# linto-ai/ssak

Hardware: AMD Instinct MI355X
Metric: utterances/sec (16 kHz, 10 s) Wav2Vec2-base CTC train step (higher is better)
Workload: dtype bf16; 1 GPU; Wav2Vec2-base CTC fine-tune step, bf16, synthetic 10 s @16 kHz utterances (BASELINE.json configs[1]; DP over xGMI for n_gpus>1 = configs[2]); per_gpu_batch=32, global_batch=32, samples_per_utt=160000, frames=499, frozen_feature_encoder=True, regularisers=script defaults (dropout/layerdrop/specaugment on), parallelism=dp1

## Files before the change

include/ssak_hip.h:

```cpp
#ifndef SSAK_HIP_H
#define SSAK_HIP_H
#include <stddef.h>
#include <stdint.h>

#ifdef __cplusplus
extern "C" {
#endif

#define SSAK_OK 0
#define SSAK_ERR_INVALID (-1)
#define SSAK_ERR_LAUNCH (-2)
#define SSAK_ERR_STATE (-3)

#define SSAK_REDUCTION_SUM 0
#define SSAK_REDUCTION_MEAN 1

int ssak_version(void);
const char* ssak_last_error(void);

size_t ssak_wave_normalize_workspace_bytes(int B, int T);
int ssak_wave_normalize(const float* in, const int32_t* lens, int B, int T, float* out, int32_t* mask,
                        void* workspace, size_t workspace_bytes, void* stream);

size_t ssak_logmel_table_floats(void);
// ... 277 lines not shown
#define SSAK_CLS_SITE_INPUT 4
#define SSAK_CLS_SITE_HIDDEN 5
int ssak_cls_head_fwd(const float* pooled, const float* W1, const float* b1, const float* W2, const float* b2, int B, int H, int C,
                      float drop_p, uint64_t seed, int training, float* act, float* logits, void* stream);
size_t ssak_cls_head_bwd_workspace_bytes(int B, int H, int C);
int ssak_cls_head_bwd(const float* dlogits, const float* pooled, const float* act, const float* W1, const float* W2, int B, int H, int C,
                      float drop_p, uint64_t seed, int training, float* dW1, float* db1, float* dW2, float* db2, float* dpooled,
                      void* workspace, size_t workspace_bytes, void* stream);
int ssak_cls_softmax_ce(const float* logits, const int32_t* labels, const int32_t* labels_host , int B, int C, float grad_scale,
                        float* probs, float* loss, float* dlogits, void* stream);

int ssak_dec_embed(const void* embed_tokens, const void* embed_positions, const int32_t* ids, const int32_t* ids_host , int B, int L,
                   int D, int V, int max_positions, int pos_offset, void* out, void* stream);
int ssak_dec_attention_fwd(const void* q, long ldq, const void* k, long ldk, const void* v, long ldv, int Lk, const int32_t* klens,
                           const int32_t* klens_host , int B, int Lq, int nh, int head_dim, int causal, int q_offset, void* ctx,
                           void* stream);
int ssak_token_logprobs(const void* logits, int dtype, int R, int V, long ldv, const int32_t* targets, const int32_t* targets_host ,
                        const int32_t* allowed, const int32_t* allowed_host , int n_allowed, float* lse, float* logprob,
                        int32_t* argmax, float* probs, void* stream);

size_t ssak_dec_attention_step_workspace_bytes(int B, int nh, int n_split);
int ssak_dec_attention_step(const void* q, long ldq, const void* k, long ldk, long k_batch_stride, const void* v, long ldv,
                            long v_batch_stride, int n_keys, const int32_t* klens, int B, int nh, int head_dim, int n_split, void* workspace,
                            size_t workspace_bytes, void* ctx, void* stream);
int ssak_dec_greedy_step(const float* logits, long ldv, int B, int V, const uint8_t* suppress, const uint8_t* begin_suppress, int first,
                         const void* embed_tokens, const void* embed_positions, int D, int max_positions, int next_pos, int eos_id, int pad_id,
                         uint8_t* finished, int32_t* n_unfinished, int32_t* tokens, float* logprobs, long ldt, int t, void* h_next,
                         void* stream);
int ssak_dec_timestamp_step(const float* logits, long ldv, int B, int V, const uint8_t* suppress, const uint8_t* begin_suppress, int first,
                            int ts_begin, int no_timestamps_id, int max_initial, const void* embed_tokens, const void* embed_positions, int D,
                            int max_positions, int next_pos, int eos_id, int pad_id, uint8_t* finished, int32_t* n_unfinished,
                            int32_t* tokens, float* logprobs, long ldt, int t, int32_t* ts_last, void* h_next, void* stream);
int ssak_dec_beam_topk(const float* logits, long ldv, int B, int nb, int V, const uint8_t* suppress, const uint8_t* begin_suppress, int first,
                       int timestamps, int ts_begin, int no_timestamps_id, int max_initial, int eos_id, const int32_t* tokens, long ldt, int t,
                       const int32_t* ts_last, const uint8_t* done, int K, int32_t* cand_token, float* cand_logprob, void* stream);
int ssak_dec_beam_select(const int32_t* cand_token, const float* cand_logprob, int B, int nb, int K, int V, float* sum_logprob, int32_t* src,
                         int32_t* tokens, float* logprobs, long ldt, int t, int32_t* ts_last, int ts_begin, int32_t* fin_tokens,
                         float* fin_logprobs, int32_t* fin_len, float* fin_sum, int32_t* n_fin, uint8_t* done, int32_t* n_unfinished,
                         const void* embed_tokens, const void* embed_positions, int D, int max_positions, int next_pos, int eos_id, int pad_id,
                         void* h_next, void* stream);
int ssak_dec_kv_reorder(void* cache, const int32_t* src, int layers, int B, int nb, int cap, int width, long layer_stride, long row_stride,
                        long key_stride, int row_lo, int row_hi, void* stream);
int ssak_dec_attention_step_grouped(const void* q, long ldq, const void* k, long ldk, long k_batch_stride, const void* v, long ldv,
                                    long v_batch_stride, int n_keys, const int32_t* klens, int B, int nh, int head_dim, int n_split, int group,
                                    void* workspace, size_t workspace_bytes, void* ctx, void* stream);
int ssak_layernorm_fwd(const void* y, const void* res, const float* gamma, const float* beta, void* r_out, void* out, int M, int C,
                       float eps, int dtype, void* stream);

int ssak_debug_dropout_mask(uint64_t seed, uint32_t site, float p, long rows, int cols, uint8_t* keep, float* scale_out ,
                            void* stream);
int ssak_debug_attention_dropout_mask(uint64_t seed, uint32_t site, float p, int B, int nh, int F, uint8_t* keep, void* stream);

int ssak_debug_layernorm_fwd(const void* y, const void* res, const float* gamma, const float* beta, void* r_out, void* out, float* mean,
                             float* rstd, int M, int C, float eps, uint64_t seed, uint32_t pre_site, float pre_p, uint32_t mid_site,
                             float mid_p, uint32_t post_site, float post_p, int post_gelu, int dtype, void* stream);
size_t ssak_debug_layernorm_bwd_workspace_bytes(int C);
int ssak_debug_layernorm_bwd(const void* g1, const void* g2, const void* r, const float* mean, const float* rstd, const float* gamma,
                             const void* g_res, void* dr, void* dy, float* dgamma, float* dbeta, float* dy_colsum,
                             const float* post_gelu_beta, int M, int C, uint64_t seed, uint32_t pre_site, float pre_p, uint32_t mid_site,
                             float mid_p, uint32_t post_site, float post_p, int queued, int dtype, void* workspace,
                             size_t workspace_bytes, void* stream);
int ssak_debug_softmax_fwd(const void* S, void* P, void* Pd, const int32_t* klens, int rows, int cols, int ld, int rows_per_batch,
                           uint64_t seed, uint32_t site, float p, int dtype, void* stream);
int ssak_debug_softmax_bwd(const void* dPd, const void* P, void* dS, int rows, int cols, int ld, uint64_t seed, uint32_t site, float p,
                           int dtype, void* stream);
int ssak_debug_gelu(const float* x, long n, float* y, float* dydx, int dtype, void* stream);

int ssak_test_attn_adapter_fwd(const void* y, const void* res, const float* ln_g, const float* ln_b, const void* w1, const float* b1,
                               const void* w2, const float* b2, const float* next_g, const float* next_b, void* r_out, void* out,
                               float* mean, float* rstd, int M, int H, int A, float eps_adapter, float eps_next, int dtype,
                               void* stream);

int ssak_debug_posconv_prepare(const float* g, const float* v, void* wf, void* wb, float* norms, int H, int G, int K, int dtype,
                               void* stream);
int ssak_debug_posconv_pack(const void* h, void* pg, int B, int F, int H, int G, int K, int dtype, void* stream);
size_t ssak_debug_posconv_workspace_bytes(int B, int F, int H, int G, int K);
int ssak_debug_posconv_direct(const void* h, const void* w, const float* bias, void* out, void* pre, int B, int F, int H, int G, int K,
                              int row0, int gelu, void* workspace, size_t workspace_bytes, void* stream);
int ssak_debug_posconv_wgrad(const void* h, const void* dpre, float* dwf, int B, int F, int H, int G, int K, void* workspace,
                             size_t workspace_bytes, void* stream);
int ssak_debug_posconv_weight_bwd(const float* dwf, const float* g, const float* v, float* norms, float* dg, float* dv, int H, int G,
                                  int K, void* stream);

size_t ssak_debug_conv0_bwd_workspace_bytes(int B, int T, int C);
int ssak_debug_conv0_bwd(const float* x, const float* w, const float* gamma, const float* beta, const void* dy, const double* sums,
                         float* dw, float* dgamma, float* dbeta, int B, int T, int C, int dtype, void* workspace, size_t workspace_bytes,
                         void* stream);
size_t ssak_debug_conv0_wgrad_workspace_bytes(int B, int C, int ksize);
int ssak_debug_conv0_wgrad(const void* d, const float* x, float* dw, int B, int T, int C, int ksize, int stride, int dtype, void* workspace,
                           size_t workspace_bytes, void* stream);
int ssak_debug_conv0_bias(const float* x, const float* w, const float* bias, void* out, int B, int T, int C, int dtype, void* stream);
int ssak_debug_col2im(const void* dxcol, void* dx, int B, int Tin, int Tout, int C, int k, int s, int dtype, void* stream);
int ssak_debug_sum_slabs(const float* slabs, int nb, long n, float* out, void* stream);
int ssak_debug_conv_weight_rearrange(const float* w, void* out, int Co, int Ci, int k, int dtype, void* stream);
int ssak_debug_conv_wgrad_unrearrange(const float* dwr, float* g, int Co, int Ci, int k, void* stream);
int ssak_debug_col2im_k3s2(const void* dxcol, const void* pre, void* out, int B, int F, int Tin, int RS1, int H, int dtype, void* stream);
int ssak_debug_mel_to_cl(const float* mel, void* cl, int B, int C, int T, int RS, int lead, int dtype, void* stream);
int ssak_debug_add_rowvec(const void* x, const void* pos, void* out, int B, int F, int H, int dtype, void* stream);
int ssak_debug_copy_rows_padded(const void* src, void* dst, int B, int F, int RS, int H, int dtype, void* stream);

#ifdef __cplusplus
}
#endif
#endif
```

ssak_amd/csrc/api.cpp:

```cpp
#include <stdarg.h>
#include <stdio.h>

#include <string.h>

#include <mutex>
#include <vector>

#include "kernels.h"

static thread_local char g_err[512] = "";

void ssak_set_error(const char* fmt, ...) {
  va_list ap;
  va_start(ap, fmt);
  vsnprintf(g_err, sizeof(g_err), fmt, ap);
  va_end(ap);
}

extern "C" int ssak_version(void) { return 630; }
extern "C" const char* ssak_last_error(void) { return g_err; }

#include <atomic>
#include <map>
namespace {
struct ProfRec {
  hipEvent_t e0, e1;
  int slot;
  double work;
};
struct ProfStream {
  int mode = 0;
  std::vector<char> want;
  std::vector<ProfRec> recs;
};
struct ProfKey {
  int dev;
  hipStream_t st;
  bool operator<(const ProfKey& o) const { return dev != o.dev ? dev < o.dev : st < o.st; }
};
std::mutex g_prof_mu;
std::map<ProfKey, ProfStream> g_prof_streams;
std::atomic<int> g_prof_active{0};
std::vector<hipEvent_t> g_event_pool;
ProfKey prof_key(hipStream_t st) {
  int dev = 0;
  (void)hipGetDevice(&dev);
  return ProfKey{dev, st};
}
hipEvent_t prof_event() {
  if (!g_event_pool.empty()) {
    hipEvent_t e = g_event_pool.back();
    g_event_pool.pop_back();
    return e;
  }
  hipEvent_t e;
  (void)hipEventCreate(&e);
  return e;
}
struct SlotInfo {
  char name[112];
  int bound;
};
SlotInfo g_slots[PROF_MAX_SLOTS];
int g_nslots = 0;
std::mutex g_slot_mu;
int register_locked(const char* name, int bound) {
  for (int i = 0; i < g_nslots; ++i)
    if (!strcmp(g_slots[i].name, name)) return i;
  if (g_nslots >= PROF_MAX_SLOTS) return PROF_MAX_SLOTS - 1;
  snprintf(g_slots[g_nslots].name, sizeof(g_slots[g_nslots].name), "%s", name);
  g_slots[g_nslots].bound = bound;
  return g_nslots++;
}
void register_classes() {
  static const struct {
    const char* name;
    int bound;
  } kClasses[PROF_CLASS_SLOTS] = {
      {"attn_fwd_kernel (fused attention forward)", SSAK_BOUND_MFMA},
      {"attn_bwd_dq_kernel + attn_bwd_dkv_kernel (fused attention backward)", SSAK_BOUND_MFMA},
      {"ln_fwd_kernel (residual + dropout + LayerNorm)", SSAK_BOUND_HBM},
      {"ln_bwd_kernel (LayerNorm backward + column partials)", SSAK_BOUND_HBM},
      {"conv0_moments_kernel + conv0_channel_stats_kernel + conv0_mfma_kernel (conv0 + GroupNorm + GELU)", SSAK_BOUND_HBM},
      {"adamw_kernel (clip + AdamW + bf16 shadow)", SSAK_BOUND_HBM},
      {"sumsq_kernel (gradient norm)", SSAK_BOUND_HBM},
      {"ctc_lsm + ctc_lat + ctc_grad (CTC loss + gradient)", SSAK_BOUND_LATENCY},
      {"norm_stats + norm_apply (waveform normalise)", SSAK_BOUND_HBM},
      {"row / element-wise helpers (pack, SpecAugment, casts, column sums, GELU', adds, reductions)", SSAK_BOUND_HBM},
      {"positional-conv weight-norm prepare / backward", SSAK_BOUND_HBM},
      {"softmax fwd / bwd (unfused attention fallback)", SSAK_BOUND_HBM},
      {"posconv_direct_kernel (grouped positional convolution forward / input gradient)", SSAK_BOUND_MFMA},
      {"posconv_wgrad_kernel + posconv_wgrad_sum_kernel (grouped positional convolution weight gradient)", SSAK_BOUND_MFMA},
      {"stft_fft_mel_kernel + logmel_finalize_kernel (Whisper log-mel features)", SSAK_BOUND_HBM},
  };
  if (g_nslots == 0)
    for (int i = 0; i < PROF_CLASS_SLOTS; ++i) register_locked(kClasses[i].name, kClasses[i].bound);
}
}

int ssak_prof_register(const char* name, int bound) {
  std::lock_guard<std::mutex> lock(g_slot_mu);
  register_classes();
// ... 87 lines not shown
```

ssak_amd/csrc/conv_frontend.hip:

```cpp
#include <cstdlib>

#include "kernels.h"

namespace {

constexpr int KS0 = 10, ST0 = 5;
constexpr int FR_STATS = 1024, FR_APPLY = 128;

template <typename OT, bool APPLY, int FR0>
__global__ __launch_bounds__(256) void conv0_kernel(const float* __restrict__ x, const float* __restrict__ w,
                                                    const float* __restrict__ gamma, const float* __restrict__ beta,
                                                    OT* __restrict__ out, double* __restrict__ stats,
                                                    const double* __restrict__ sums, int T, int T0, int C) {
  constexpr int NS0 = (FR0 - 1) * ST0 + KS0;
  __shared__ float xs[NS0];
  __shared__ float red[256][9];
  const int b = blockIdx.y;
  const int f0 = blockIdx.x * FR0;
  const int nq = C >> 2;
  const int fl = 256 / nq;
  const int q = threadIdx.x % nq, fli = threadIdx.x / nq;
  const int nfr = min(FR0, T0 - f0);
  const float* xb = x + (size_t)b * T;
  for (int i = threadIdx.x; i < NS0; i += 256) {
// ... 648 lines not shown
  }
  float* out = partial + ((size_t)b * gridDim.x + blk) * C * ksize;
  const int c2 = threadIdx.x;
  if (c2 < C / 2)
#pragma unroll
    for (int k = 0; k < 10; ++k)
      if (k < ksize) {
        out[(2 * c2) * ksize + k] = acc[0][k];
        out[(2 * c2 + 1) * ksize + k] = acc[1][k];
      }
}
__global__ void conv0_wgrad_sum_kernel(const float* __restrict__ partial, int nslab, int n, float* __restrict__ dw) {
  const int e = blockIdx.x * blockDim.x + threadIdx.x;
  if (e >= n) return;
  float s = 0.f;
  for (int k = 0; k < nslab; ++k) s += partial[(size_t)k * n + e];
  dw[e] += s;
}

}

size_t k_conv0_wgrad_scratch_floats(int B, int C, int ksize) { return (size_t)B * C0W_BLOCKS_PER_UTT * C * ksize; }

template <typename DT>
int k_conv0_wgrad_t(const DT* d, const float* x, float* dw, float* scratch, int B, int T, int T0, int C, int ksize, int stride,
                    hipStream_t st) {
  SSAK_REQUIRE(ksize <= 10 && stride * 64 + ksize <= 64 * 5 + 16 && C <= 512 && (C & 1) == 0,
               "conv0_wgrad: kernel %d / stride %d / C %d outside what is built (k <= 10, stride <= 5, C <= 512)", ksize, stride, C);
  conv0_wgrad_kernel<DT><<<dim3(C0W_BLOCKS_PER_UTT, B), 256, 0, st>>>(d, x, scratch, T, T0, C, ksize, stride);
  SSAK_LAUNCH_CHECK();
  conv0_wgrad_sum_kernel<<<ssak_cdiv(C * ksize, 256), 256, 0, st>>>(scratch, B * C0W_BLOCKS_PER_UTT, C * ksize, dw);
  SSAK_LAUNCH_CHECK();
  return SSAK_OK;
}

size_t k_conv0_stats_doubles(int B, int T0, int C) {
  return (size_t)B * 2 * C + (size_t)B * ssak_cdiv(T0, FR_STATS) * std::max(2 * C, NMOM);
}

template <typename OT>
int k_conv0_gn_gelu_t(const float* x, const float* w, const float* gamma, const float* beta, OT* out, double* stats,
                      int B, int T, int T0, int C, int ksize, int stride, hipStream_t st, bool raw_input) {
  SSAK_REQUIRE(ksize == KS0 && stride == ST0, "conv0: only kernel 10 / stride 5 is built (got %d/%d)", ksize, stride);
  SSAK_REQUIRE((C & 3) == 0 && C <= 1024 && 256 % (C / 4) == 0, "conv0: C=%d must divide into 256 threads as quads", C);
  SSAK_REQUIRE(T0 == (T - KS0) / ST0 + 1 && T0 > 0, "conv0: T0 mismatch");
  const int nblk = ssak_cdiv(T0, FR_STATS);
  ProfScope prof_scope(PROF_CONV0, (double)B * ((double)T * 4.0 + (double)T0 * C * sizeof(OT)), st);
  double* sums = stats;
  double* partial = stats + (size_t)B * 2 * C;
  conv0_moments_kernel<<<dim3(nblk, B), 256, 0, st>>>(x, T, T0, partial);
  SSAK_LAUNCH_CHECK();
  conv0_channel_stats_kernel<<<dim3(ssak_cdiv(C, 256), B), 256, 0, st>>>(partial, nblk, w, C, sums, T, T0, raw_input ? 1 : 0);
  SSAK_LAUNCH_CHECK();
  if constexpr (sizeof(OT) == 2) {
    if (C == 512) {
      conv0_mfma_kernel<<<dim3(ssak_cdiv(T0, C0M_FR * C0M_SUB), B), 256, 0, st>>>(x, w, gamma, beta, (bf16*)out, sums, T, T0);
      SSAK_LAUNCH_CHECK();
      return SSAK_OK;
    }
  }
  conv0_kernel<OT, true, FR_APPLY><<<dim3(ssak_cdiv(T0, FR_APPLY), B), 256, 0, st>>>(x, w, gamma, beta, out, nullptr, sums, T, T0, C);
  SSAK_LAUNCH_CHECK();
  return SSAK_OK;
}

template <typename OT>
int k_conv0_bias_t(const float* x, const float* w, const float* bias, OT* out, int B, int T, int T0, int C, int ksize,
                   int stride, hipStream_t st) {
  SSAK_REQUIRE(ksize == KS0 && stride == ST0, "conv0: only kernel 10 / stride 5 is built (got %d/%d)", ksize, stride);
  SSAK_REQUIRE((C & 3) == 0 && C <= 1024 && 256 % (C / 4) == 0, "conv0: C=%d must divide into 256 threads as quads", C);
  ProfScope prof_scope(PROF_CONV0, (double)B * ((double)T * 4.0 + (double)T0 * C * sizeof(OT)), st);
  conv0_bias_kernel<OT><<<dim3(ssak_cdiv(T0, FR_APPLY), B), 256, 0, st>>>(x, w, bias, out, T, T0, C);
  SSAK_LAUNCH_CHECK();
  return SSAK_OK;
}

template <typename OT>
int k_conv_weight_rearrange_t(const float* w, OT* out, int Co, int Ci, int k, hipStream_t st) {
  conv_w_rearrange_kernel<OT><<<min(2048, ssak_cdiv((long)Co * Ci * k, 256)), 256, 0, st>>>(w, out, Co, Ci, k);
  SSAK_LAUNCH_CHECK();
  return SSAK_OK;
}

template <typename OT>
int k_posconv_prepare_t(const float* g, const float* v, OT* w_fwd, OT* w_bwd, float* norms, int H, int G, int K,
                        hipStream_t st) {
  SSAK_REQUIRE(K <= 1024 && H % G == 0 && ((H / G) & 7) == 0, "posconv: K=%d <= 1024 and (H/G)=%d %% 8 == 0 required", K, H / G);
  const int cg = H / G;
  float* partial = norms + 2 * K;
  ProfScope prof_scope(PROF_POSCONV_W, (double)H * cg * K * 8.0, st);
  posconv_colnorm_kernel<<<H, ((K + 63) / 64) * 64, 0, st>>>(v, nullptr, H / cg, K, cg, partial);
  SSAK_LAUNCH_CHECK();
  posconv_colnorm_finalize_kernel<<<ssak_cdiv(K, 64), 1024, 0, st>>>(partial, H, K, norms);
  SSAK_LAUNCH_CHECK();
  SSAK_REQUIRE((size_t)cg * (K + 1) * sizeof(float) <= 64 * 1024, "posconv: (H/G) x K slab does not fit in LDS");
  posconv_materialize_kernel<OT><<<2 * H, 256, (size_t)cg * (K + 1) * sizeof(float), st>>>(g, v, norms, w_fwd, w_bwd, H, cg, K);
  SSAK_LAUNCH_CHECK();
  return SSAK_OK;
}

int k_posconv_weight_bwd(const float* dw, const float* g, const float* v, const float* norms, float* dg, float* dv,
                         int H, int G, int K, hipStream_t st) {
  const int cg = H / G;
  float* dot = const_cast<float*>(norms) + K;
  float* partial = const_cast<float*>(norms) + 2 * K;
  ProfScope prof_scope(PROF_POSCONV_W, (double)H * cg * K * 12.0, st);
  posconv_colnorm_kernel<<<H, ((K + 63) / 64) * 64, 0, st>>>(v, dw, H / cg, K, cg, partial);
  SSAK_LAUNCH_CHECK();
  posconv_colnorm_finalize_kernel<<<ssak_cdiv(K, 64), 1024, 0, st>>>(partial, H, K, dot);
  SSAK_LAUNCH_CHECK();
  SSAK_REQUIRE((size_t)K * (cg + 1) * sizeof(float) <= 64 * 1024, "posconv: K x (H/G) slab does not fit in LDS");
  posconv_wbwd_kernel<<<H, 256, (size_t)K * (cg + 1) * sizeof(float), st>>>(dw, g, v, norms, dot, dg, dv, H, cg, K);
  SSAK_LAUNCH_CHECK();
  return SSAK_OK;
}

template <typename T>
int k_posconv_pack_t(const T* h, T* pg, int B, int F, int H, int G, int K, hipStream_t st) {
  const int lead = K / 2, RS = F + K;
  const long rows_total = lead + (long)B * RS + K;
  const long n = rows_total * G * (H / G / 8);
  ProfScope prof_scope(PROF_ROWWISE, (double)B * F * H * 2.0 * sizeof(T), st);
  posconv_pack_kernel<T><<<min(4096, ssak_cdiv(n, 256)), 256, 0, st>>>(h, pg, B, F, H, G, lead, RS, rows_total);
  SSAK_LAUNCH_CHECK();
  return SSAK_OK;
}

template <typename T_>
int k_col2im_t(const T_* dxcol, T_* dx, int B, int Tin, int Tout, int C, int k, int s, hipStream_t st) {
  SSAK_REQUIRE((C & 7) == 0, "col2im: C must be a multiple of 8");
  const long n8 = (long)B * Tin * C / 8;
  col2im_kernel<T_><<<min(8192, ssak_cdiv(n8, 256)), 256, 0, st>>>(dxcol, dx, Tin, Tout, C, k, s, n8);
  SSAK_LAUNCH_CHECK();
  return SSAK_OK;
}

int k_sum_slabs(const float* slabs, int nb, long n, float* out, hipStream_t st) {
  sum_slabs_kernel<<<min(4096, ssak_cdiv(n, 256)), 256, 0, st>>>(slabs, nb, n, out);
  SSAK_LAUNCH_CHECK();
  return SSAK_OK;
}

size_t k_conv0_bwd_scratch_floats(int B, int T0, int C) {
  const size_t nblk = ssak_cdiv(T0, FR_STATS);
  return (size_t)B * nblk * (C / 4) * (4 * KS0) + (size_t)B * C * 2 * 2  + 64;
}

template <typename DT>
int k_conv0_gn_gelu_bwd_t(const float* x, const float* w, const float* gamma, const float* beta, const DT* dy,
                          const double* sums, float* scratch, float* dw, float* dgamma, float* dbeta, int B, int T, int T0, int C,
                          hipStream_t st) {
  SSAK_REQUIRE((C & 3) == 0 && C <= 1024 && 256 % (C / 4) == 0, "conv0_bwd: C=%d must divide into 256 threads as quads", C);
  const int nblk = ssak_cdiv(T0, FR_STATS);
  double* gsums = reinterpret_cast<double*>(scratch);
  float* partial = scratch + (size_t)B * C * 2 * 2 + 16;
  dim3 grid(nblk, B);
  conv0_bwd_kernel<0, DT><<<grid, 256, 256 * 9 * sizeof(float), st>>>(x, w, gamma, beta, dy, sums, nullptr, partial, T, T0, C);
  SSAK_LAUNCH_CHECK();
  conv0_bwd_gsums_kernel<<<dim3(ssak_cdiv(2 * C, 256), B), 256, 0, st>>>(partial, nblk, C, gsums);
  SSAK_LAUNCH_CHECK();
  conv0_bwd_affine_kernel<<<ssak_cdiv(C, 256), 256, 0, st>>>(gsums, B, C, dgamma, dbeta);
  SSAK_LAUNCH_CHECK();
  constexpr int lds1 = 256 * (4 * KS0 + 1) * sizeof(float);
  static bool attr_done = false;
  if (!attr_done) {
    SSAK_HIP(hipFuncSetAttribute((const void*)conv0_bwd_kernel<1, DT>, hipFuncAttributeMaxDynamicSharedMemorySize, lds1));
    attr_done = true;
  }
  conv0_bwd_kernel<1, DT><<<grid, 256, lds1, st>>>(x, w, gamma, beta, dy, sums, gsums, partial, T, T0, C);
  SSAK_LAUNCH_CHECK();
  conv0_bwd_dw_kernel<<<ssak_cdiv(C * KS0, 256), 256, 0, st>>>(partial, B * nblk, C, dw);
  SSAK_LAUNCH_CHECK();
  return SSAK_OK;
}

#define SSAK_INSTANTIATE_CONV_KERNELS(T)                                                                                       \
  template int k_conv0_gn_gelu_t<T>(const float*, const float*, const float*, const float*, T*, double*, int, int, int, int,   \
// ... 140 lines not shown
```

ssak_amd/csrc/kernels.h:

```cpp
#pragma once
#include "common.h"

enum : int {
  PROF_ATTN_FWD = 0, PROF_ATTN_BWD, PROF_LN_FWD, PROF_LN_BWD, PROF_CONV0, PROF_ADAMW, PROF_SUMSQ, PROF_CTC, PROF_WAVE_NORM,
  PROF_ROWWISE, PROF_POSCONV_W, PROF_SOFTMAX, PROF_POSCONV_DIRECT, PROF_POSCONV_WGRAD, PROF_LOGMEL,
  PROF_CLASS_SLOTS
};
constexpr int PROF_MAX_SLOTS = 128;
int ssak_prof_register(const char* name, int bound);
bool ssak_prof_wanted(int slot, hipStream_t st);
class ProfScope {
 public:
  ProfScope(int slot, double work, hipStream_t st);
  ~ProfScope();
  ProfScope(const ProfScope&) = delete;
  ProfScope& operator=(const ProfScope&) = delete;

 private:
  hipStream_t st_;
  hipEvent_t e0_ = nullptr;
  int slot_;
  double work_;
  bool on_;
};
// ... 16 lines not shown
  int n = 0;
  bool push(const float* partial, long stride, int slots, int ncols, float* out) {
    if (n >= CAP) return false;
    jobs[n++] = ReduceJob{partial, out, stride, slots, ncols};
    return true;
  }
};
extern thread_local ReduceSink* g_reduce_sink;
int k_reduce_flush(ReduceSink& sink, hipStream_t st);

template <typename T>
int k_layernorm_fwd_t(const T* y, const T* res, const float* gamma, const float* beta, T* r_out, T* out,
                      float* mean, float* rstd, int M, int C, float eps, const DropSpec& pre, const DropSpec& post,
                      hipStream_t st, const DropSpec& mid = DropSpec(), bool post_gelu = false);
template <typename T>
int k_layernorm_bwd_t(const T* g1, const T* g2, const T* r, const float* mean, const float* rstd,
                      const float* gamma, const T* g_res, T* dr, T* dy, float* dgamma, float* dbeta,
                      float* partial , int M, int C, const DropSpec& pre, const DropSpec& post,
                      hipStream_t st, const DropSpec& mid = DropSpec(), float* dy_colsum = nullptr ,
                      const float* post_gelu_beta = nullptr );
#ifndef SSAK_LN_BWD_BLOCKS
#define SSAK_LN_BWD_BLOCKS 768
#endif
#ifndef SSAK_LN_FWD_BLOCKS
#define SSAK_LN_FWD_BLOCKS 768
#endif
constexpr int LN_FWD_BLOCKS = SSAK_LN_FWD_BLOCKS;
constexpr int LN_BWD_BLOCKS = SSAK_LN_BWD_BLOCKS;
template <typename T>
int k_softmax_fwd_t(const T* S, T* P, T* Pd, const int32_t* klens, int rows, int cols, int ld,
                    int rows_per_batch, const DropSpec& drop, hipStream_t st);
template <typename T>
int k_softmax_bwd_t(const T* dPd, const T* P, T* dS, int rows, int cols, int ld, const DropSpec& drop,
                    hipStream_t st);
template <typename T>
int k_colsum_t(const T* X, long ld, int M, int N, float* out, hipStream_t st, float* scratch = nullptr, size_t scratch_floats = 0,
               const uint8_t* rowmask = nullptr, const int32_t* flens = nullptr, int F = 0);
int k_cast_f32_bf16(const float* in, bf16* out, long n, hipStream_t st);
template <typename T>
int k_specaug_fwd_t(T* h, const uint8_t* mask, const int32_t* flens, const float* embed, int B, int F, int C,
                    hipStream_t st);
template <typename T>
int k_specaug_bwd_t(T* dh, const uint8_t* mask, const int32_t* flens, float* dembed, int B, int F, int C,
                    hipStream_t st, float* scratch = nullptr, size_t scratch_floats = 0);
template <typename T>
int k_gelu_grad_mul_t(const T* dy, const T* pre, T* out, long n, hipStream_t st);
template <typename T>
int k_add_t(const T* a, const T* b, T* out, long n, hipStream_t st);
int k_layernorm_fwd(const bf16* y, const bf16* res, const float* gamma, const float* beta, bf16* r_out, bf16* out,
                    float* mean, float* rstd, int M, int C, float eps, const DropSpec& pre, const DropSpec& post,
                    hipStream_t st, const DropSpec& mid = DropSpec(), bool post_gelu = false);
int k_layernorm_bwd(const bf16* g1, const bf16* g2, const bf16* r, const float* mean, const float* rstd,
                    const float* gamma, const bf16* g_res, bf16* dr, bf16* dy, float* dgamma, float* dbeta,
                    float* partial, int M, int C, const DropSpec& pre, const DropSpec& post,
                    hipStream_t st, const DropSpec& mid = DropSpec(), float* dy_colsum = nullptr,
                    const float* post_gelu_beta = nullptr);
int k_colsum(const bf16* X, long ld, int M, int N, float* out, hipStream_t st, float* scratch = nullptr, size_t scratch_floats = 0,
             const uint8_t* rowmask = nullptr, const int32_t* flens = nullptr, int F = 0);

size_t k_conv0_stats_doubles(int B, int T0, int C);
template <typename T>
int k_conv0_gn_gelu_t(const float* x, const float* w, const float* gamma, const float* beta, T* out, double* stats,
                      int B, int Tn, int T0, int C, int ksize, int stride, hipStream_t st, bool raw_input = false);
size_t k_conv0_wgrad_scratch_floats(int B, int C, int ksize);
template <typename DT>
int k_conv0_wgrad_t(const DT* d, const float* x, float* dw, float* scratch, int B, int T, int T0, int C, int ksize, int stride,
                  hipStream_t st);
template <typename T>
int k_conv0_bias_t(const float* x, const float* w, const float* bias, T* out, int B, int Tn, int T0, int C, int ksize,
                   int stride, hipStream_t st);
template <typename T_>
int k_col2im_t(const T_* dxcol, T_* dx, int B, int Tin, int Tout, int C, int k, int s, hipStream_t st);
int k_sum_slabs(const float* slabs, int nb, long n, float* out, hipStream_t st);
size_t k_conv0_bwd_scratch_floats(int B, int T0, int C);
template <typename DT>
int k_conv0_gn_gelu_bwd_t(const float* x, const float* w, const float* gamma, const float* beta, const DT* dy,
                        const double* sums, float* scratch, float* dw, float* dgamma, float* dbeta, int B, int T, int T0, int C,
                        hipStream_t st);
template <typename T>
int k_conv_weight_rearrange_t(const float* w, T* out, int Co, int Ci, int k, hipStream_t st);
template <typename T>
int k_posconv_prepare_t(const float* g, const float* v, T* w_fwd, T* w_bwd, float* norms, int H, int G, int K,
                        hipStream_t st);
int k_posconv_weight_bwd(const float* dw, const float* g, const float* v, const float* norms, float* dg, float* dv,
                         int H, int G, int K, hipStream_t st);
template <typename T>
int k_posconv_pack_t(const T* h, T* pg, int B, int F, int H, int G, int K, hipStream_t st);

bool k_attn_adapter_supported(int H, int A);
template <typename T>
int k_attn_adapter_fwd_t(const T* y, const T* res, const float* ln_g, const float* ln_b, const T* w1, const float* b1, const T* w2,
                         const float* b2, const float* next_g, const float* next_b, T* r_out, T* out, float* mean, float* rstd, int M,
                         int H, int A, float eps_adapter, float eps_next, hipStream_t st);

bool k_attention_supported(int H, int nh);
int k_attention_fwd(const bf16* qkv, bf16* ctx, float* lse, const int32_t* klens, int B, int F, int nh, int H,
                    const DropSpec& drop, hipStream_t st);
size_t k_attention_bwd_bias_floats(int B, int F, int H);
int k_attention_bwd(const bf16* qkv, const bf16* ctx, const float* lse, const int32_t* klens, const bf16* dctx, float* delta,
                    bf16* dqkv, int B, int F, int nh, int H, const DropSpec& drop, int mode , hipStream_t st,
                    float* bias_part = nullptr, float* bias_grad = nullptr);
int k_colsum_rows(const float* partial, int slots, int N, float* out, hipStream_t st);

bool k_posconv_direct_supported(int H, int G, int K);
int k_posconv_frag_weights(const bf16* w, bf16* wfrag, int H, int G, int K, hipStream_t st);
int k_posconv_direct(const bf16* x, long rows_per_group, int row0, const bf16* w, const float* bias, bf16* out, bf16* pre, int B, int F,
                     int H, int G, int K, int gelu, hipStream_t st);

size_t k_posconv_wgrad_scratch_floats(int H, int G, int K);
int k_posconv_wgrad_direct(const bf16* x, const bf16* dy, long rows_per_group, long rows, int lead, float* dwf, float* scratch, int H, int G,
                           int K, hipStream_t st);

template <typename T_>
int k_mel_to_cl_t(const float* mel, T_* cl, int B, int C, int T, int RS, int lead, hipStream_t st);
template <typename T_>
int k_add_rowvec_t(const T_* x, const T_* pos, T_* out, int B, int F, int H, hipStream_t st);
template <typename T_>
int k_copy_rows_padded_t(const T_* src, T_* dst, int B, int F, int RS, int H, hipStream_t st);
template <typename T_>
int k_col2im_k3s2_t(const T_* dxcol, const T_* pre, T_* out, int B, int F, int Tin, int RS1, int H, hipStream_t st);
int k_conv_wgrad_unrearrange(const float* dwr, float* g, int Co, int Ci, int k, hipStream_t st);

int k_sumsq(const float* g, long n, float* out , float* partial, hipStream_t st, bool add = false );
int k_adamw(float* p, const float* g, float* m, float* v, bf16* shadow, long n, const float* gnorm_sq, float max_norm,
            float grad_scale, float lr, float beta1, float beta2, float eps, float wd, int step, hipStream_t st);

int ssak_gemm_p8_launch(const void* params, int bm, int a_km, int b_km, hipStream_t st);
int k_transpose_bf16_batched(int n, const bf16* const* src, bf16* const* dst, const int* R, const int* C, hipStream_t st);

int ssak_gemm_ticket_slot(hipStream_t st, int** out);
bool ssak_gemm_p4_supports(const void* params, int bm, int a_km, int b_km);
int ssak_gemm_p4_launch(const void* params, int bm, int b_km, hipStream_t st);
int ssak_gemm_p8bd_launch(const void* params, int bm, hipStream_t st);
size_t k_gemm_fragment_b_bytes(int N, int K);
int k_gemm_fragment_b_batched(int n, const void* const* B, const long* ldb, const int* N, const int* K, const int* b_km, void* const* out,
                              hipStream_t st);
int ssak_gemm_p8_launch_grouped(const void* params, int n, const void* const* A, const void* const* B, void* const* C, const int* M,
                                const int* N, const long* lda, const long* ldb, const long* ldc, const uint32_t* ext_a,
                                const uint32_t* ext_b, int a_km, int b_km, hipStream_t st);
```

ssak_amd/csrc/posconv.hip:

```cpp
#include <algorithm>

#include "common.h"
#include "kernels.h"

namespace {

constexpr int PC_TM = 512;
constexpr int PC_WROWS = 128;

template <int CG>
struct PcGeom {
  static constexpr int TP = CG == 48 ? 2 : 1;
  static constexpr int KK = TP * CG / 32;
  static constexpr int NJ = CG / 16;
  static constexpr int CPR = CG / 8;
  static constexpr int PITCH = CG == 48 ? 96 : 160;
};

struct PcParams {
  const bf16* x;
  const bf16* w;
  const float* bias;
  bf16* out;
  bf16* pre;
// ... 76 lines not shown
  load_b(b1, s + 1);
  __builtin_amdgcn_sched_barrier(0);
  compute(b0, s);
  __builtin_amdgcn_sched_barrier(0);
  compute(b1, s + 1);
  const int col0 = grp * CG + 4 * g4;
#pragma unroll
  for (int i = 0; i < 8; ++i) {
    const int t = t0 + wave * PC_WROWS + 16 * i + lc;
    if (t >= p.F) continue;
    const long o = ((long)b * p.F + t) * p.H + col0;
#pragma unroll
    for (int j = 0; j < NJ; ++j) {
      float v[4];
#pragma unroll
      for (int r = 0; r < 4; ++r) v[r] = acc[i][j][r] + (p.bias ? p.bias[col0 + 16 * j + r] : 0.f);
      if (p.pre) {
        const bf16x4 q = {(bf16)v[0], (bf16)v[1], (bf16)v[2], (bf16)v[3]};
        *reinterpret_cast<bf16x4*>(p.pre + o + 16 * j) = q;
      }
      if (p.gelu) {
        const f32x2 y0 = gelu2((f32x2){v[0], v[1]}), y1 = gelu2((f32x2){v[2], v[3]});
        v[0] = y0[0], v[1] = y0[1], v[2] = y1[0], v[3] = y1[1];
      }
      const bf16x4 q = {(bf16)v[0], (bf16)v[1], (bf16)v[2], (bf16)v[3]};
      *reinterpret_cast<bf16x4*>(p.out + o + 16 * j) = q;
    }
  }
}

template <int CG>
__global__ void posconv_frag_kernel(const bf16* __restrict__ w, bf16* __restrict__ wfrag, int G, int K) {
  using G_ = PcGeom<CG>;
  const long nchunks = (long)G * CG * K * CG / 8;
  for (long c = (long)blockIdx.x * blockDim.x + threadIdx.x; c < nchunks; c += (long)gridDim.x * blockDim.x) {
    const int lane = (int)(c & 63);
    long r = c >> 6;
    const int kk = (int)(r % G_::KK);
    r /= G_::KK;
    const int j = (int)(r % G_::NJ);
    r /= G_::NJ;
    const int nsteps = K / G_::TP;
    const int step = (int)(r % nsteps), g = (int)(r / nsteps);
    const int lc = lane & 15, g4 = lane >> 4;
    const bf16* src = w + ((long)g * CG + 16 * j + lc) * ((long)K * CG) + (long)step * G_::TP * CG + 32 * kk + 8 * g4;
    *reinterpret_cast<uint4*>(wfrag + c * 8) = *reinterpret_cast<const uint4*>(src);
  }
}

template <int CG>
int launch_posconv(const PcParams& p, hipStream_t st) {
  const size_t lds = (size_t)(PC_TM + p.K - 1 + 1) * PcGeom<CG>::PITCH;
  static bool attr_done = false;
  if (!attr_done) {
    SSAK_HIP(hipFuncSetAttribute((const void*)posconv_direct_kernel<CG>, hipFuncAttributeMaxDynamicSharedMemorySize, 160 * 1024));
    attr_done = true;
  }
  posconv_direct_kernel<CG><<<dim3(ssak_cdiv(p.F, PC_TM), p.H / CG, p.B), 256, lds, st>>>(p);
  SSAK_LAUNCH_CHECK();
  return SSAK_OK;
}

}

bool k_posconv_direct_supported(int H, int G, int K) {
  const int cg = G > 0 ? H / G : 0;
  if (G <= 0 || H % G || (cg != 48 && cg != 64)) return false;
  if (K < 4 || (K & (cg == 48 ? 3 : 1))) return false;
  return (size_t)(PC_TM + K) * (cg == 48 ? 96 : 160) <= 150 * 1024;
}

int k_posconv_frag_weights(const bf16* w, bf16* wfrag, int H, int G, int K, hipStream_t st) {
  SSAK_REQUIRE(k_posconv_direct_supported(H, G, K), "posconv_frag_weights: H=%d G=%d K=%d not built", H, G, K);
  const long nchunks = (long)H * K * (H / G) / 8;
  const int grid = (int)std::min<long>(4096, (nchunks + 255) / 256);
  if (H / G == 48)
    posconv_frag_kernel<48><<<grid, 256, 0, st>>>(w, wfrag, G, K);
  else
    posconv_frag_kernel<64><<<grid, 256, 0, st>>>(w, wfrag, G, K);
  SSAK_LAUNCH_CHECK();
  return SSAK_OK;
}

int k_posconv_direct(const bf16* x, long rows_per_group, int row0, const bf16* w, const float* bias, bf16* out, bf16* pre, int B, int F,
                     int H, int G, int K, int gelu, hipStream_t st) {
  SSAK_REQUIRE(k_posconv_direct_supported(H, G, K), "posconv_direct: H=%d G=%d K=%d not built", H, G, K);
  PcParams p{x, w, bias, out, pre, rows_per_group, (long)F + K, row0, B, F, H, K, gelu};
  ProfScope prof_scope(PROF_POSCONV_DIRECT, 2.0 * B * F * (double)H * K * (H / G), st);
  return H / G == 48 ? launch_posconv<48>(p, st) : launch_posconv<64>(p, st);
}

namespace {

constexpr int PW_RB = 128;
constexpr int PW_SPLIT = 4;
template <int CG>
struct PwGeom {
  static constexpr int CB = CG / 16;
  static constexpr int TW = CG == 48 ? 4 : 2;
  static constexpr int TT = 4 * TW;
  static constexpr int XR = PW_RB + TT - 1;
  static constexpr int CPR = CG / 8;
  static constexpr int NCH = (XR + PW_RB) * CPR;
  static constexpr int PER_T = (NCH + 255) / 256;
};
struct PwParams {
  const bf16* x;
  const bf16* dy;
  float* part;
  long rows_per_group;
  long rows;
  int lead, K, G;
};
__device__ __forceinline__ int pw_swz(int r) { return ((r >> 1) & 1) | (((r >> 3) & 1) << 1); }

template <int CG>
__global__ __launch_bounds__(256, 2) void posconv_wgrad_kernel(const PwParams p) {
  using G_ = PwGeom<CG>;
  constexpr int CB = G_::CB, TW = G_::TW, TT = G_::TT, CPR = G_::CPR;
  constexpr int XP = (G_::XR + 7) / 8, YP = PW_RB / 8;
  constexpr int XROWS = 8 * XP;
  constexpr int BUF = (XROWS + PW_RB) * 128;
  extern __shared__ __attribute__((aligned(16))) char img[];
  const int lane = threadIdx.x & 63, wave = __builtin_amdgcn_readfirstlane(threadIdx.x >> 6);
  const int tb = blockIdx.x, grp = blockIdx.y, split = blockIdx.z;
  const long per_split = ((p.rows + PW_RB - 1) / PW_RB + PW_SPLIT - 1) / PW_SPLIT * PW_RB;
  const long r_lo = (long)split * per_split, r_hi = min(p.rows, r_lo + per_split);
  const uint32_t ext = (uint32_t)(p.rows_per_group * CG * 2);
  const __amdgpu_buffer_rsrc_t xr = __builtin_amdgcn_make_buffer_rsrc((void*)(p.x + (long)grp * p.rows_per_group * CG), 0, (int)ext, 0x00020000);
  const __amdgpu_buffer_rsrc_t yr = __builtin_amdgcn_make_buffer_rsrc((void*)(p.dy + (long)grp * p.rows_per_group * CG), 0, (int)ext, 0x00020000);
  typedef __attribute__((address_space(3))) void lds_void_;
  uint32_t src_off[2];
#pragma unroll
  for (int par = 0; par < 2; ++par) {
    const int r = 8 * par + (lane >> 3), s16 = lane & 7;
    const int ch = 2 * ((s16 >> 1) ^ pw_swz(r)) + (s16 & 1);
    src_off[par] = ch < CPR ? (uint32_t)(((lane >> 3) * CG + ch * 8) * 2) : 0x80000000u;
  }
  auto stage = [&](char* buf, long rb) {
    const long x0 = rb + (long)tb * TT, y0 = (long)p.lead + rb;
#pragma unroll
    for (int i = 0; i < (XP + YP + 3) / 4; ++i) {
      const int pc = wave + 4 * i;
      if (pc < XP + YP) {
        const bool is_x = pc < XP;
        const int ip = is_x ? pc : pc - XP;
        const long row0 = (is_x ? x0 : y0) + 8 * ip;
        const uint32_t so = src_off[ip & 1];
        const uint32_t o = so == 0x80000000u ? so : (uint32_t)(row0 * CG * 2) + so;
        __builtin_amdgcn_raw_ptr_buffer_load_lds(is_x ? xr : yr, (lds_void_*)(buf + (is_x ? 0 : XROWS * 128) + ip * 1024), 16, o, 0, 0, 0);
      }
    }
  };
  const int g4 = lane >> 4, q4 = (lane >> 2) & 3, p4 = lane & 3;
  typedef __attribute__((address_space(3))) char lds_char;
  const uint32_t img_a = (uint32_t)(uintptr_t)(lds_char*)img;
  uint32_t xrow[TW][2], xsw[TW][2], yrow[2], ysw[2];
#pragma unroll
  for (int hi = 0; hi < 2; ++hi) {
    const int kr = 8 * g4 + q4 + 4 * hi;
    yrow[hi] = img_a + (XROWS + kr) * 128 + 8 * p4;
    ysw[hi] = pw_swz(kr) << 5;
#pragma unroll
    for (int tw = 0; tw < TW; ++tw) {
      const int row = kr + wave * TW + tw;
      xrow[tw][hi] = img_a + row * 128 + 8 * p4;
// ... 106 lines not shown
    if (!attr48) {
      SSAK_HIP(hipFuncSetAttribute((const void*)posconv_wgrad_kernel<48>, hipFuncAttributeMaxDynamicSharedMemorySize, (int)lds));
      attr48 = true;
    }
    posconv_wgrad_kernel<48><<<dim3(K / PwGeom<48>::TT, G, PW_SPLIT), 256, lds, st>>>(p);
  } else {
    SSAK_REQUIRE(K % PwGeom<64>::TT == 0, "posconv_wgrad_direct: K must be a multiple of %d", PwGeom<64>::TT);
    constexpr size_t lds = 2 * (size_t)((PwGeom<64>::XR + 7) / 8 * 8 + PW_RB) * 128;
    static bool attr64 = false;
    if (!attr64) {
      SSAK_HIP(hipFuncSetAttribute((const void*)posconv_wgrad_kernel<64>, hipFuncAttributeMaxDynamicSharedMemorySize, (int)lds));
      attr64 = true;
    }
    posconv_wgrad_kernel<64><<<dim3(K / PwGeom<64>::TT, G, PW_SPLIT), 256, lds, st>>>(p);
  }
  SSAK_LAUNCH_CHECK();
  const long n4 = (long)H * K * cg / 4;
  posconv_wgrad_sum_kernel<<<(int)std::min<long>(2048, (n4 + 255) / 256), 256, 0, st>>>(scratch, dwf, n4);
  SSAK_LAUNCH_CHECK();
  return SSAK_OK;
}

namespace {
struct PcDebugWs {
  size_t x, dy, frag, scratch, total;
  long rows_per_group;
};
bool pc_debug_geometry(int B, int F, int H, int G, int K) {
  return B > 0 && F > 0 && k_posconv_direct_supported(H, G, K) && K % (H / G == 48 ? PwGeom<48>::TT : PwGeom<64>::TT) == 0 &&
         (long)B * F < (1L << 30);
}
PcDebugWs pc_debug_ws(int B, int F, int H, int G, int K) {
  auto up = [](size_t n) { return (n + 255) / 256 * 256; };
  PcDebugWs w;
  w.rows_per_group = K / 2 + (long)B * (F + K) + K;
  const size_t packed = up((size_t)G * w.rows_per_group * (H / G) * sizeof(bf16));
  w.x = 0;
  w.dy = packed;
  w.frag = 2 * packed;
  w.scratch = w.frag + up((size_t)H * K * (H / G) * sizeof(bf16));
  w.total = w.scratch + up(k_posconv_wgrad_scratch_floats(H, G, K) * sizeof(float));
  return w;
}
}

extern "C" size_t ssak_debug_posconv_workspace_bytes(int B, int F, int H, int G, int K) {
  return pc_debug_geometry(B, F, H, G, K) ? pc_debug_ws(B, F, H, G, K).total : 0;
}

extern "C" int ssak_debug_posconv_direct(const void* h, const void* w, const float* bias, void* out, void* pre, int B, int F, int H, int G,
                                         int K, int row0, int gelu, void* workspace, size_t workspace_bytes, void* stream) {
  SSAK_REQUIRE(h && w && out && workspace, "debug_posconv_direct: null pointer");
  SSAK_REQUIRE(pc_debug_geometry(B, F, H, G, K), "debug_posconv_direct: B=%d F=%d H=%d G=%d K=%d not built", B, F, H, G, K);
  SSAK_REQUIRE(row0 >= 0 && row0 <= 1, "debug_posconv_direct: row0=%d (0 forward, 1 input gradient)", row0);
  const PcDebugWs ws = pc_debug_ws(B, F, H, G, K);
  SSAK_REQUIRE(workspace_bytes >= ws.total, "debug_posconv_direct: workspace too small");
  const hipStream_t st = (hipStream_t)stream;
  char* base = (char*)workspace;
  bf16* px = (bf16*)(base + ws.x);
  bf16* frag = (bf16*)(base + ws.frag);
  int rc = k_posconv_pack_t<bf16>((const bf16*)h, px, B, F, H, G, K, st);
  if (rc != SSAK_OK) return rc;
  rc = k_posconv_frag_weights((const bf16*)w, frag, H, G, K, st);
  if (rc != SSAK_OK) return rc;
  return k_posconv_direct(px, ws.rows_per_group, row0, frag, bias, (bf16*)out, (bf16*)pre, B, F, H, G, K, gelu != 0, st);
}

extern "C" int ssak_debug_posconv_wgrad(const void* h, const void* dpre, float* dwf, int B, int F, int H, int G, int K, void* workspace,
                                        size_t workspace_bytes, void* stream) {
  SSAK_REQUIRE(h && dpre && dwf && workspace, "debug_posconv_wgrad: null pointer");
  SSAK_REQUIRE(pc_debug_geometry(B, F, H, G, K), "debug_posconv_wgrad: B=%d F=%d H=%d G=%d K=%d not built", B, F, H, G, K);
  const PcDebugWs ws = pc_debug_ws(B, F, H, G, K);
  SSAK_REQUIRE(workspace_bytes >= ws.total, "debug_posconv_wgrad: workspace too small");
  const hipStream_t st = (hipStream_t)stream;
  char* base = (char*)workspace;
  bf16* px = (bf16*)(base + ws.x);
  bf16* pdy = (bf16*)(base + ws.dy);
  int rc = k_posconv_pack_t<bf16>((const bf16*)h, px, B, F, H, G, K, st);
  if (rc != SSAK_OK) return rc;
  rc = k_posconv_pack_t<bf16>((const bf16*)dpre, pdy, B, F, H, G, K, st);
  if (rc != SSAK_OK) return rc;
  return k_posconv_wgrad_direct(px, pdy, ws.rows_per_group, (long)B * (F + K), K / 2, dwf, (float*)(base + ws.scratch), H, G, K, st);
}
```

ssak_amd/csrc/w2v2_engine.hip:

```cpp
#include <algorithm>
#include <string>
#include <vector>
#include <string.h>

#include "kernels.h"
#include "wgrad_schedule.h"

namespace {

struct PInfo {
  std::string name;
  std::vector<long> shape;
  long offset = 0, numel = 0;
  int region = 0;
};

struct LayerP {
  long wqkv, bqkv, wo, bo, ln1w, ln1b, w1, b1, w2, b2, ln2w, ln2b;
  long ad_nw = 0, ad_nb = 0, ad_w1 = 0, ad_b1 = 0, ad_w2 = 0, ad_b2 = 0;
};

inline long align_up(long x, long a) { return (x + a - 1) / a * a; }

struct Carver {
  size_t off = 0;
  size_t take(size_t bytes) {
    const size_t o = off;
    off = (size_t)align_up((long)(off + bytes), 256);
    return o;
  }
};

struct LayerBuf {
  size_t qkv, P, Pd, ctx, r1, x1, f1pre, f1, r2, st;
  size_t lse;
};

struct Plan {
  int B = 0, T = 0, F = 0, M = 0, Fp = 0, training = 0;
  int Tl[8] = {0};
  long pg_rows = 0;
  size_t bufA, bufB, feat, stats0, ln0, st0, h0, pgx, pc_pre, pc, h1, stE, tmpH, S, xf, flens;
  std::vector<size_t> x;
  std::vector<LayerBuf> lb;
  size_t dlog, dA, dB, dY, dC, dI, dqkv, dSb, pgdy, dwf, slab, dln0, scratchH, lnpart, redring, redring_floats;
  size_t dY1 = 0, dYb[WGRAD_SETS] = {0}, dIb[WGRAD_SETS] = {0}, dqkvb[WGRAD_SETS] = {0}, dY1b[WGRAD_SETS] = {0};
  int Tin = 0, RS1 = 0, RS2 = 0;
  bool fused_attn = false;
  size_t delta = 0;
  bool fe_train = false;
  size_t act[8] = {0}, cpre[8] = {0}, fe_dp = 0, fe_da = 0, fe_db = 0, fe_dxcol = 0, fe_slab = 0, fe_dwr = 0, fe_c0 = 0;
  size_t fe_st[8] = {0};
  size_t melcl, h1pad, pre1, wpre2, we, dpre2pad, dxcol, dpre1pad, dwr;
  size_t slab_bytes = 0;
  size_t total = 0;
};

}

struct ssak_w2v2 {
  ssak_w2v2_config cfg;
  std::vector<PInfo> params;
  long n_total = 0, n_train = 0;
  long p_mse, p_fpln_w, p_fpln_b, p_fp_w, p_fp_b, p_pc_b, p_pc_g, p_pc_v, p_eln_w, p_eln_b, p_lm_w, p_lm_b;
  long p_conv_w[8], p_conv_b[8], p_cln_w[8], p_cln_b[8];
  long p_c1w = 0, p_c1b = 0, p_c2w = 0, p_c2b = 0, p_pos = 0;
  std::vector<size_t> hres;
  std::vector<LayerP> lp;
  float* P = nullptr;
  float* G = nullptr;
  bf16* W = nullptr;
  void* conv_w[8] = {nullptr};
  void* pc_wf = nullptr;
  void* pc_wb = nullptr;
  bf16* pc_wf_frag = nullptr;
  bf16* pc_wb_frag = nullptr;
  float* pc_norms = nullptr;
  Plan plan;
  bool have_fwd = false;
  bool fwd_hidden = false;
  uint64_t seed = 0;
  const uint8_t* spec_mask = nullptr;
  const int32_t* lens = nullptr;
  const float* last_input = nullptr;
  std::vector<int> keep;
  ssak_grad_ready_fn on_ready = nullptr;
  void* on_ready_user = nullptr;
  hipEvent_t params_ready = nullptr, stall_begin = nullptr, stall_end = nullptr;
  int dynamic_tiles = 0;
  size_t xin[SSAK_MAX_LAYERS + 1] = {0};
  int raw_input = 0;
  int attn_bwd_mode = SSAK_ATTN_BWD_DEFAULT;
  int posconv_direct = 1;
  int fragment_weights = 0;
  bf16* wfrag = nullptr;
  size_t wfrag_layer = 0;
  size_t wfrag_off[6] = {0};
  bool wfrag_use[6] = {false};
  int wfrag_M = 0;
  bool wfrag_valid = false;
  const bf16* frag(int layer, int which) const {
    return (wfrag_valid && wfrag_use[which] && keep[layer]) ? wfrag + (size_t)layer * wfrag_layer + wfrag_off[which] : nullptr;
  }
  int transposed_weights = 1;
  bf16* wtr = nullptr;
  size_t wtr_layer = 0;
  size_t wtr_off[4] = {0};
  bool wtr_valid = false;
  const bf16* wt(int layer, int which) const {
    return (wtr_valid && keep[layer]) ? wtr + (size_t)layer * wtr_layer + wtr_off[which] : nullptr;
  }
  long layer_span() const { return (lp[0].w2 + (long)cfg.hidden_size * cfg.intermediate_size) - lp[0].wqkv; }
  long n_grad() const { return (cfg.arch == 1 || cfg.freeze_feature_encoder) ? n_train : n_total; }
};

namespace {

enum : uint32_t { DS_FEATPROJ = 1, DS_ENCIN = 2, DS_FINAL = 3, DS_LAYER0 = 16 };
inline uint32_t ds_attn(int l) { return DS_LAYER0 + 4 * l; }
inline uint32_t ds_hid1(int l) { return DS_LAYER0 + 4 * l + 1; }
inline uint32_t ds_act(int l) { return DS_LAYER0 + 4 * l + 2; }
inline uint32_t ds_hid2(int l) { return DS_LAYER0 + 4 * l + 3; }

int conv_len(int L, int k, int s) { return (L - k) / s + 1; }

void add_param(ssak_w2v2* e, long& cursor, const std::string& name, std::vector<long> shape, int region, long* off_out) {
  PInfo pi;
  pi.name = name;
  pi.shape = shape;
  pi.numel = 1;
  for (long d : shape) pi.numel *= d;
  pi.offset = cursor;
  pi.region = region;
  cursor = align_up(cursor + pi.numel, 8);
  if (off_out) *off_out = pi.offset;
  e->params.push_back(pi);
}

void build_param_table_whisper(ssak_w2v2* e) {
  const ssak_w2v2_config& c = e->cfg;
  const long H = c.hidden_size, I = c.intermediate_size, V = c.vocab_size, NM = c.num_mel_bins;
  long cur = 0, dummy;
  e->lp.resize(c.num_layers);
  add_param(e, cur, "encoder.conv1.weight", {H, NM, 3}, 0, &e->p_c1w);
  add_param(e, cur, "encoder.conv2.weight", {H, H, 3}, 0, &e->p_c2w);
  for (int l = 0; l < c.num_layers; ++l) {
    const std::string p = "encoder.layers." + std::to_string(l) + ".";
    LayerP& L = e->lp[l];
    add_param(e, cur, p + "self_attn.q_proj.weight", {H, H}, 0, &L.wqkv);
    add_param(e, cur, p + "self_attn.k_proj.weight", {H, H}, 0, &dummy);
    add_param(e, cur, p + "self_attn.v_proj.weight", {H, H}, 0, &dummy);
    add_param(e, cur, p + "self_attn.out_proj.weight", {H, H}, 0, &L.wo);
    add_param(e, cur, p + "fc1.weight", {I, H}, 0, &L.w1);
    add_param(e, cur, p + "fc2.weight", {H, I}, 0, &L.w2);
  }
  add_param(e, cur, "ctc_head.weight", {V, H}, 0, &e->p_lm_w);
  add_param(e, cur, "encoder.conv1.bias", {H}, 0, &e->p_c1b);
  add_param(e, cur, "encoder.conv2.bias", {H}, 0, &e->p_c2b);
  for (int l = 0; l < c.num_layers; ++l) {
// ... 644 lines not shown
    return SSAK_ERR_INVALID;
  }
  return SSAK_OK;
}

extern "C" int ssak_w2v2_set_grad_ready_callback(ssak_w2v2* e, ssak_grad_ready_fn fn, void* user) {
  SSAK_REQUIRE(e, "w2v2_set_grad_ready_callback: null handle");
  e->on_ready = fn;
  e->on_ready_user = user;
  return SSAK_OK;
}

extern "C" int ssak_w2v2_grad_ranges(const ssak_w2v2_config* cfg, long* offsets, long* counts, int cap) {
  SSAK_REQUIRE(cfg && offsets && counts && cap > 0, "w2v2_grad_ranges: null pointer");
  TRY(check_config(*cfg));
  ssak_w2v2 e;
  e.cfg = *cfg;
  build_param_table(&e);
  const ssak_w2v2_config& c = e.cfg;
  const long H = c.hidden_size, V = c.vocab_size;
  int n = 0;
  auto put = [&](long off, long cnt) {
    if (cnt <= 0) return;
    if (n < cap) {
      offsets[n] = off;
      counts[n] = cnt;
    }
    ++n;
  };
  put(e.p_lm_w, V * H);
  for (int l = c.num_layers - 1; l >= 0; --l) put(e.lp[l].wqkv, e.layer_span());
  put(0, e.lp[0].wqkv);
  put(e.p_lm_w + V * H, e.n_grad() - (e.p_lm_w + V * H));
  return n;
}

extern "C" int ssak_w2v2_set_param_event(ssak_w2v2* e, void* params_ready, void* stall_begin, void* stall_end) {
  SSAK_REQUIRE(e, "w2v2_set_param_event: null handle");
  e->params_ready = (hipEvent_t)params_ready;
  e->stall_begin = (hipEvent_t)stall_begin;
  e->stall_end = (hipEvent_t)stall_end;
  return SSAK_OK;
}

extern "C" int ssak_w2v2_sync_weights(ssak_w2v2* e, int full, void* stream) {
  SSAK_REQUIRE(e && e->P && e->W, "w2v2_sync_weights: bind the parameter buffers first");
  hipStream_t st = (hipStream_t)stream;
  const ssak_w2v2_config& c = e->cfg;
  if (c.arch == 1) {
    if (full) TRY(k_cast_f32_bf16(e->P, e->W, e->n_total, st));
    if (c.exact) {
      TRY(k_conv_weight_rearrange_t<float>(e->P + e->p_c1w, (float*)e->conv_w[1], c.hidden_size, c.num_mel_bins, 3, st));
      TRY(k_conv_weight_rearrange_t<float>(e->P + e->p_c2w, (float*)e->conv_w[2], c.hidden_size, c.hidden_size, 3, st));
    } else {
      TRY(k_conv_weight_rearrange_t<bf16>(e->P + e->p_c1w, (bf16*)e->conv_w[1], c.hidden_size, c.num_mel_bins, 3, st));
      TRY(k_conv_weight_rearrange_t<bf16>(e->P + e->p_c2w, (bf16*)e->conv_w[2], c.hidden_size, c.hidden_size, 3, st));
    }
    return SSAK_OK;
  }
  if (full) {
    TRY(k_cast_f32_bf16(e->P, e->W, e->n_total, st));
    long cin = c.conv_dim[0];
    for (int i = 1; i < c.num_conv_layers; ++i) {
      if (c.exact)
        TRY(k_conv_weight_rearrange_t<float>(e->P + e->p_conv_w[i], (float*)e->conv_w[i], c.conv_dim[i], (int)cin, c.conv_kernel[i], st));
      else
        TRY(k_conv_weight_rearrange_t<bf16>(e->P + e->p_conv_w[i], (bf16*)e->conv_w[i], c.conv_dim[i], (int)cin, c.conv_kernel[i], st));
      cin = c.conv_dim[i];
    }
  }
  if (!full && !c.freeze_feature_encoder) {
    long cin2 = c.conv_dim[0];
    for (int i = 1; i < c.num_conv_layers; ++i) {
      if (c.exact)
        TRY(k_conv_weight_rearrange_t<float>(e->P + e->p_conv_w[i], (float*)e->conv_w[i], c.conv_dim[i], (int)cin2, c.conv_kernel[i], st));
      else
        TRY(k_conv_weight_rearrange_t<bf16>(e->P + e->p_conv_w[i], (bf16*)e->conv_w[i], c.conv_dim[i], (int)cin2, c.conv_kernel[i], st));
      cin2 = c.conv_dim[i];
    }
  }
  if (c.exact)
    TRY(k_posconv_prepare_t<float>(e->P + e->p_pc_g, e->P + e->p_pc_v, (float*)e->pc_wf, (float*)e->pc_wb, e->pc_norms, c.hidden_size,
                                   c.num_conv_pos_embedding_groups, c.num_conv_pos_embeddings, st));
  else {
    TRY(k_posconv_prepare_t<bf16>(e->P + e->p_pc_g, e->P + e->p_pc_v, (bf16*)e->pc_wf, (bf16*)e->pc_wb, e->pc_norms, c.hidden_size,
                                  c.num_conv_pos_embedding_groups, c.num_conv_pos_embeddings, st));
    if (e->pc_wf_frag) {
      TRY(k_posconv_frag_weights((const bf16*)e->pc_wf, e->pc_wf_frag, c.hidden_size, c.num_conv_pos_embedding_groups, c.num_conv_pos_embeddings, st));
      TRY(k_posconv_frag_weights((const bf16*)e->pc_wb, e->pc_wb_frag, c.hidden_size, c.num_conv_pos_embedding_groups, c.num_conv_pos_embeddings, st));
    }
  }
  return SSAK_OK;
}

extern "C" size_t ssak_w2v2_workspace_bytes(const ssak_w2v2* e, int B, int T, int training) {
  if (!e || B <= 0 || T <= 0) return 0;
  Plan p;
  if (make_plan(e, B, T, training, p) != SSAK_OK) return 0;
  return p.total;
}

extern "C" int ssak_w2v2_num_frames(const ssak_w2v2* e, int T) {
  if (!e) return 0;
  if (e->cfg.arch == 1) return (T >= 2 && (T & 1) == 0) ? T / 2 : 0;
  int L = T;
  for (int i = 0; i < e->cfg.num_conv_layers; ++i) {
    if (L < e->cfg.conv_kernel[i]) return 0;
    L = conv_len(L, e->cfg.conv_kernel[i], e->cfg.conv_stride[i]);
  }
  return L;
}

template <typename AT>
struct Call {
  static constexpr bool EXACT = sizeof(AT) == 4;
  ssak_w2v2* const e;
  const ssak_w2v2_config& c;
  const Plan& p;
  char* const ws;
  const hipStream_t st;
  const bool tr;
  const uint64_t seed;
  const bool whisper, stable;
  const int H, I, V, nh, hd, nc, C, K, G, cg, B, F, M, Fp;
  const float* const P;
  float* const Gd;
  const AT* const W;
  int32_t* const flens;
  const float scale;
  const DropSpec none;
  void* const slab;
  const size_t cs_floats;

  Call(ssak_w2v2* e_, void* workspace, void* stream, bool training)
      : e(e_), c(e_->cfg), p(e_->plan), ws((char*)workspace), st((hipStream_t)stream), tr(training), seed(e_->seed),
        whisper(c.arch == 1), stable(whisper || c.do_stable_layer_norm != 0), H(c.hidden_size), I(c.intermediate_size),
        V(c.vocab_size), nh(c.num_heads), hd(H / nh), nc(whisper ? 1 : c.num_conv_layers), C(whisper ? 8 : c.conv_dim[nc - 1]),
        K(whisper ? 8 : c.num_conv_pos_embeddings), G(whisper ? 1 : c.num_conv_pos_embedding_groups), cg(H / G), B(p.B), F(p.F),
        M(p.M), Fp(p.Fp), P(e_->P), Gd(e_->G), W(EXACT ? (const AT*)e_->P : (const AT*)e_->W),
        flens(e_->lens ? (int32_t*)(ws + p.flens) : nullptr), scale(1.f / sqrtf((float)hd)), slab(ws + p.slab),
        cs_floats((size_t)LN_BWD_BLOCKS * 3 * std::max(H, C)) {}

  AT* BF(size_t off) const { return (AT*)(ws + off); }
  float* FP(size_t off) const { return (float*)(ws + off); }
  DropSpec DS(float prob, uint32_t stream_id) const {
    DropSpec d;
    d.seed = seed;
    d.stream = stream_id;
    d.p = tr ? prob : 0.f;
    return d;
  }
  long next_ln_w(int l) const { return (l + 1 < c.num_layers) ? e->lp[l + 1].ln1w : e->p_eln_w; }
  long next_ln_b(int l) const { return (l + 1 < c.num_layers) ? e->lp[l + 1].ln1b : e->p_eln_b; }

  bool waited = false;
  int wait_params();
  int fwd_whisper_frontend(const float* input_values);
  int fwd_features(const float* input_values, const int32_t* lens, int32_t* frame_lens);
  int fwd_posconv_encoder_input();
  int fwd_layer(int l, bool skip);
  int fwd_head(float* logits, void* hidden);

  AT* gA = nullptr;
  AT* gB = nullptr;
  const AT* Gres = nullptr;
  int kept = 0;
  AT* free_buf(const AT* u1, const AT* u2, const AT* u3) const {
    AT* cand[3] = {BF(p.dC), BF(p.dA), BF(p.scratchH)};
    for (AT* cnd : cand)
      if (cnd != u1 && cnd != u2 && cnd != u3) return cnd;
    return (AT*)nullptr;
  }
  void announce(long off, long cnt) const { WgradAnnounce{e}(off, cnt); }
  int bwd_zero_grads();
// ... 24 lines not shown
  SSAK_HIP(hipMemsetAsync(ws + p.h1pad, 0, ((size_t)B * RS1 + 8) * H * sizeof(AT), st));
  TRY(k_mel_to_cl_t<AT>(input_values, BF(p.melcl), B, NM, Tin, RS1, 1, st));
  TRY(GemmX<EXACT>(Tin, H, 3 * NM).a(BF(p.melcl), NM).b(e->conv_w[1], 3 * NM).c(BF(p.h1pad) + H, H)
          .batch(B, 1, (long)RS1 * NM, 0, 0, 0, (long)RS1 * H, 0).with_bias(P + e->p_c1b)
          .epi(SSAK_EPI_GELU, nullptr, BF(p.pre1) + H).run(st));
  TRY(GemmX<EXACT>(F, H, 3 * H).a(BF(p.h1pad), 2 * H).b(e->conv_w[2], 3 * H).c(BF(p.we), H)
          .batch(B, 1, (long)RS1 * H, 0, 0, 0, (long)F * H, 0).with_bias(P + e->p_c2b)
          .epi(SSAK_EPI_GELU, nullptr, BF(p.wpre2)).run(st));
  TRY(k_add_rowvec_t<AT>(BF(p.we), W + e->p_pos, BF(p.h1), B, F, H, st));
  TRY(k_layernorm_fwd_t<AT>(BF(p.h1), nullptr, P + e->lp[0].ln1w, P + e->lp[0].ln1b, BF(p.h1), BF(p.x[0]), FP(p.stE),
                      FP(p.stE) + M, M, H, c.layer_norm_eps, none, none, st, DS(c.hidden_dropout, DS_ENCIN)));
  return SSAK_OK;
}

template <typename AT>
int Call<AT>::fwd_features(const float* input_values, const int32_t* lens, int32_t* frame_lens) {
  const int T = p.T;
  if (lens) {
    ConvChain cc;
    cc.n = nc;
    for (int i = 0; i < nc; ++i) {
      cc.k[i] = c.conv_kernel[i];
      cc.s[i] = c.conv_stride[i];
    }
    frame_lens_kernel<<<ssak_cdiv(B, 64), 64, 0, st>>>(lens, B, T, cc, flens);
    SSAK_LAUNCH_CHECK();
    if (frame_lens) SSAK_HIP(hipMemcpyAsync(frame_lens, flens, (size_t)B * sizeof(int32_t), hipMemcpyDeviceToDevice, st));
  }

  const bool ln_fe = c.feat_extract_norm == 1;
  SSAK_REQUIRE(!(e->raw_input && p.fe_train), "w2v2_forward: raw input (normalisation folded into conv0's GroupNorm) needs the frozen feature encoder");
  if (!ln_fe) {
    TRY(k_conv0_gn_gelu_t<AT>(input_values, P + e->p_conv_w[0], P + e->p_cln_w[0], P + e->p_cln_b[0],
                        p.fe_train ? BF(p.act[0]) : BF(p.bufA), (double*)(ws + p.stats0), B, T, p.Tl[0], c.conv_dim[0],
                        c.conv_kernel[0], c.conv_stride[0], st, e->raw_input != 0));
  } else {
    AT* pre0 = p.fe_train ? BF(p.cpre[0]) : BF(p.bufA);
    TRY(k_conv0_bias_t<AT>(input_values, P + e->p_conv_w[0], c.conv_bias ? P + e->p_conv_b[0] : nullptr, pre0, B, T,
                     p.Tl[0], c.conv_dim[0], c.conv_kernel[0], c.conv_stride[0], st));
    TRY(k_layernorm_fwd_t<AT>(pre0, nullptr, P + e->p_cln_w[0], P + e->p_cln_b[0], nullptr, p.fe_train ? BF(p.act[0]) : BF(p.bufA),
                        p.fe_train ? FP(p.fe_st[0]) : nullptr, p.fe_train ? FP(p.fe_st[0]) + (size_t)B * p.Tl[0] : nullptr,
                        B * p.Tl[0], c.conv_dim[0], 1e-5f, none, none, st, none, true));
  }
  {
    AT* src = p.fe_train ? BF(p.act[0]) : BF(p.bufA);
    for (int i = 1; i < nc; ++i) {
      AT* dst = (i == nc - 1) ? BF(p.feat) : (p.fe_train ? BF(p.act[i]) : ((i & 1) ? BF(p.bufB) : BF(p.bufA)));
      const int Ci = c.conv_dim[i - 1], Co = c.conv_dim[i], k = c.conv_kernel[i], s = c.conv_stride[i];
      AT* conv_out = (ln_fe && p.fe_train) ? BF(p.cpre[i]) : dst;
      GemmX<EXACT> g(p.Tl[i], Co, k * Ci);
      g.a(src, (long)s * Ci).b(e->conv_w[i], (long)k * Ci).c(conv_out, Co)
          .batch(B, 1, (long)p.Tl[i - 1] * Ci, 0, 0, 0, (long)p.Tl[i] * Co, 0);
      if (c.conv_bias) g.with_bias(P + e->p_conv_b[i]);
      if (!ln_fe) g.epi(SSAK_EPI_GELU, nullptr, p.fe_train ? BF(p.cpre[i]) : nullptr);
      TRY(g.run(st));
      if (ln_fe)
        TRY(k_layernorm_fwd_t<AT>(conv_out, nullptr, P + e->p_cln_w[i], P + e->p_cln_b[i], nullptr, dst,
                            p.fe_train ? FP(p.fe_st[i]) : nullptr, p.fe_train ? FP(p.fe_st[i]) + (size_t)B * p.Tl[i] : nullptr,
                            B * p.Tl[i], Co, 1e-5f, none, none, st, none, true));
      src = dst;
    }
  }
  TRY(wait_params());
  TRY(k_layernorm_fwd_t<AT>(BF(p.feat), nullptr, P + e->p_fpln_w, P + e->p_fpln_b, nullptr, BF(p.ln0), FP(p.st0),
                      FP(p.st0) + M, M, C, c.layer_norm_eps, none, none, st));
  TRY(GemmX<EXACT>(M, H, C).a(BF(p.ln0), C).b(W + e->p_fp_w, C).c(BF(p.h0), H).with_bias(P + e->p_fp_b)
          .run(st));
    if (tr && c.feat_proj_dropout > 0.f)
      TRY(k_layernorm_fwd_t<AT>(BF(p.h0), nullptr, nullptr, nullptr, BF(p.h0), nullptr, nullptr, nullptr, M, H, 0.f,
                          DS(c.feat_proj_dropout, DS_FEATPROJ), none, st));
  TRY(k_specaug_fwd_t<AT>(BF(p.h0), e->spec_mask, flens, P + e->p_mse, B, F, H, st));
  return SSAK_OK;
}

template <typename AT>
int Call<AT>::fwd_posconv_encoder_input() {
  TRY(k_posconv_pack_t<AT>(BF(p.h0), BF(p.pgx), B, F, H, G, K, st));
  bool pc_direct = false;
  if constexpr (!EXACT) pc_direct = e->posconv_direct && e->pc_wf_frag != nullptr;
  if (pc_direct) {
    if constexpr (!EXACT)
      TRY(k_posconv_direct(BF(p.pgx), p.pg_rows, 0, e->pc_wf_frag, P + e->p_pc_b, BF(p.pc), BF(p.pc_pre), B, F, H, G, K, 1, st));
  } else {
    TRY(GemmX<EXACT>(F, cg, K * cg)
            .a(BF(p.pgx), cg)
            .b(e->pc_wf, (long)K * cg)
            .c(BF(p.pc), H)
            .batch(B, G, (long)(F + K) * cg, p.pg_rows * cg, 0, (long)cg * K * cg, (long)F * H, cg)
            .with_bias(P + e->p_pc_b, cg)
            .epi(SSAK_EPI_GELU, nullptr, BF(p.pc_pre))
            .run(st));
  }
  if (!stable) {
    TRY(k_layernorm_fwd_t<AT>(BF(p.pc), BF(p.h0), P + e->p_eln_w, P + e->p_eln_b, BF(p.h1), BF(p.x[0]), FP(p.stE), FP(p.stE) + M,
                        M, H, c.layer_norm_eps, none, DS(c.hidden_dropout, DS_ENCIN), st));
  } else {
    TRY(k_layernorm_fwd_t<AT>(BF(p.pc), BF(p.h0), P + e->lp[0].ln1w, P + e->lp[0].ln1b, BF(p.h1), BF(p.x[0]), FP(p.stE),
                        FP(p.stE) + M, M, H, c.layer_norm_eps, none, none, st, DS(c.hidden_dropout, DS_ENCIN)));
  }
  return SSAK_OK;
}

template <typename AT>
int Call<AT>::fwd_layer(int l, bool skip) {
  const LayerP& L = e->lp[l];
  const LayerBuf& lb = p.lb[l];
  float* stl = FP(lb.st);
  const float* nxt_w = P + next_ln_w(l);
  const float* nxt_b = P + next_ln_b(l);
  if (skip) {
    e->keep[l] = 0;
    if (!stable) {
      e->xin[l + 1] = e->xin[l];
    } else {
      TRY(k_layernorm_fwd_t<AT>(BF(e->hres[l]), nullptr, nxt_w, nxt_b, nullptr, BF(p.x[l + 1]), stl + 2 * M, stl + 3 * M, M, H,
                          c.layer_norm_eps, none, none, st));
      e->hres[l + 1] = e->hres[l];
      e->xin[l + 1] = p.x[l + 1];
    }
    return SSAK_OK;
  }
  const AT* x = BF(e->xin[l]);
  e->xin[l + 1] = p.x[l + 1];
  AT* qkv = BF(lb.qkv);
  TRY(GemmX<EXACT>(M, 3 * H, H).a(x, H).b(W + L.wqkv, H).bfrag(e->frag(l, 0)).c(qkv, 3 * H).with_bias(P + L.bqkv).run(st));
  if (p.fused_attn) {
    if constexpr (!EXACT)
      TRY(k_attention_fwd(qkv, BF(lb.ctx), FP(lb.lse), flens, B, F, nh, H, DS(c.attention_dropout, ds_attn(l)), st));
  } else {
    TRY(GemmX<EXACT>(F, F, hd).a(qkv, 3 * H).b(qkv + H, 3 * H).c(BF(p.S), Fp).alpha(scale)
            .batch(B, nh, (long)F * 3 * H, hd, (long)F * 3 * H, hd, (long)nh * F * Fp, (long)F * Fp).run(st));
    TRY(k_softmax_fwd_t<AT>(BF(p.S), BF(lb.P), lb.Pd != lb.P ? BF(lb.Pd) : nullptr, flens, B * nh * F, F, Fp, nh * F,
                      DS(c.attention_dropout, ds_attn(l)), st));
    TRY(GemmX<EXACT>(F, hd, F).a(BF(lb.Pd), Fp).b(qkv + 2 * H, 3 * H, true).c(BF(lb.ctx), H)
            .batch(B, nh, (long)nh * F * Fp, (long)F * Fp, (long)F * 3 * H, hd, (long)F * H, hd).run(st));
  }
  TRY(GemmX<EXACT>(M, H, H).a(BF(lb.ctx), H).b(W + L.wo, H).bfrag(e->frag(l, 1)).c(BF(p.tmpH), H).with_bias(P + L.bo).run(st));
  if (!stable) {
    TRY(k_layernorm_fwd_t<AT>(BF(p.tmpH), x, P + L.ln1w, P + L.ln1b, BF(lb.r1), BF(lb.x1), stl, stl + M, M, H,
                        c.layer_norm_eps, DS(c.hidden_dropout, ds_hid1(l)), none, st));
  } else {
    TRY(k_layernorm_fwd_t<AT>(BF(p.tmpH), BF(e->hres[l]), P + L.ln2w, P + L.ln2b, BF(lb.r1), BF(lb.x1), stl, stl + M, M, H,
                        c.layer_norm_eps, DS(c.hidden_dropout, ds_hid1(l)), none, st));
  }
  TRY(GemmX<EXACT>(M, I, H).a(BF(lb.x1), H).b(W + L.w1, H).c(BF(lb.f1), I).with_bias(P + L.b1)
          .epi(tr ? SSAK_EPI_GELU_SAVE_GRAD : SSAK_EPI_GELU, nullptr, tr ? BF(lb.f1pre) : nullptr)
          .drop(tr ? c.activation_dropout : 0.f, ds_act(l), seed).run(st));
  TRY(GemmX<EXACT>(M, H, I).a(BF(lb.f1), I).b(W + L.w2, I).bfrag(e->frag(l, 2)).c(BF(p.tmpH), H).with_bias(P + L.b2).run(st));
  if (!stable) {
    TRY(k_layernorm_fwd_t<AT>(BF(p.tmpH), BF(lb.x1), P + L.ln2w, P + L.ln2b, BF(lb.r2), BF(p.x[l + 1]), stl + 2 * M, stl + 3 * M,
                        M, H, c.layer_norm_eps, DS(c.hidden_dropout, ds_hid2(l)), none, st));
  } else {
    if (c.adapter_attn_dim > 0)
      TRY(k_attn_adapter_fwd_t<AT>(BF(p.tmpH), BF(lb.r1), P + L.ad_nw, P + L.ad_nb, W + L.ad_w1, P + L.ad_b1, W + L.ad_w2, P + L.ad_b2,
                                   nxt_w, nxt_b, BF(lb.r2), BF(p.x[l + 1]), stl + 2 * M, stl + 3 * M, M, H, c.adapter_attn_dim, 1e-5f,
                                   c.layer_norm_eps, st));
    else
      TRY(k_layernorm_fwd_t<AT>(BF(p.tmpH), BF(lb.r1), nxt_w, nxt_b, BF(lb.r2), BF(p.x[l + 1]), stl + 2 * M, stl + 3 * M, M, H,
                          c.layer_norm_eps, DS(c.hidden_dropout, ds_hid2(l)), none, st));
    e->hres[l + 1] = lb.r2;
  }
  return SSAK_OK;
}

template <typename AT>
int Call<AT>::fwd_head(float* logits, void* hidden) {
  const AT* xl = BF(e->xin[c.num_layers]);
  if (hidden) {
    SSAK_HIP(hipMemcpyAsync(hidden, xl, (size_t)M * H * sizeof(AT), hipMemcpyDeviceToDevice, st));
    e->have_fwd = tr;
    e->fwd_hidden = true;
    return SSAK_OK;
  }
  e->fwd_hidden = false;
  if (tr && c.final_dropout > 0.f) {
    TRY(k_layernorm_fwd_t<AT>(xl, nullptr, nullptr, nullptr, BF(p.xf), nullptr, nullptr, nullptr, M, H, 0.f,
                        DS(c.final_dropout, DS_FINAL), none, st));
    xl = BF(p.xf);
  }
  TRY(GemmX<EXACT>(M, V, H).a(xl, H).b(W + e->p_lm_w, H).c(logits, V, true).with_bias(P + e->p_lm_b).run(st));
  e->have_fwd = tr;
  return SSAK_OK;
}

template <typename AT>
static int forward_impl(ssak_w2v2* e, const float* input_values, const int32_t* lens, int B, int T, const uint8_t* spec_mask,
                        const uint8_t* layer_keep , uint64_t seed, int training, float* logits, void* hidden ,
                        int32_t* frame_lens, void* workspace, size_t workspace_bytes, void* stream) {
  SSAK_REQUIRE(e && input_values && (logits || hidden) && workspace, "w2v2_forward: null pointer");
  SSAK_REQUIRE(e->P && e->W, "w2v2_forward: bind + sync_weights first");
  SSAK_REQUIRE(B > 0 && T > 0, "w2v2_forward: bad shape B=%d T=%d", B, T);
  SSAK_REQUIRE(((uintptr_t)workspace & 255) == 0, "w2v2_forward: workspace must be 256-byte aligned");
  SSAK_REQUIRE(!(training && e->cfg.adapter_attn_dim > 0),
               "w2v2_forward: a model with language adapters (adapter_attn_dim > 0) runs inference only: training is not implemented");
  EngineCall engine_call(e);
  e->have_fwd = false;
  TRY(make_plan(e, B, T, training, e->plan));
  SSAK_REQUIRE(workspace_bytes >= e->plan.total, "w2v2_forward: workspace too small (%zu < %zu)", workspace_bytes, e->plan.total);
  e->seed = seed;
  e->spec_mask = spec_mask;
  e->lens = lens;
  e->last_input = input_values;
  Call<AT> k(e, workspace, stream, training != 0);
  const ssak_w2v2_config& c = e->cfg;
  if (k.whisper || !c.freeze_feature_encoder) TRY(k.wait_params());
  if (k.whisper) {
    TRY(k.fwd_whisper_frontend(input_values));
  } else {
    TRY(k.fwd_features(input_values, lens, frame_lens));
    TRY(k.fwd_posconv_encoder_input());
  }
  e->keep.assign(c.num_layers, 1);
  e->wfrag_valid = false;
  if constexpr (!Call<AT>::EXACT) {
    if (k.tr && e->fragment_weights) TRY(refresh_weight_fragments(e, k.M, layer_keep, k.st));
  }
  e->wtr_valid = false;
  if constexpr (!Call<AT>::EXACT) {
    if (k.tr && e->transposed_weights && c.hidden_size % 256 == 0 && c.intermediate_size % 256 == 0) TRY(refresh_weight_transposes(e, layer_keep, k.st));
  }
  e->hres.assign(c.num_layers + 1, k.p.h1);
  e->xin[0] = k.p.x[0];
  for (int l = 0; l < c.num_layers; ++l) TRY(k.fwd_layer(l, k.tr && layer_keep && !layer_keep[l]));
  return k.fwd_head(logits, hidden);
}

extern "C" int ssak_w2v2_forward(ssak_w2v2* e, const float* input_values, const int32_t* lens, int B, int T,
                                 const uint8_t* spec_mask, const uint8_t* layer_keep , uint64_t seed,
                                 int training, float* logits, int32_t* frame_lens, void* workspace,
                                 size_t workspace_bytes, void* stream) {
  SSAK_REQUIRE(e && logits, "w2v2_forward: null pointer");
  if (e->cfg.exact)
    return forward_impl<float>(e, input_values, lens, B, T, spec_mask, layer_keep, seed, training, logits, nullptr, frame_lens, workspace,
                               workspace_bytes, stream);
  return forward_impl<bf16>(e, input_values, lens, B, T, spec_mask, layer_keep, seed, training, logits, nullptr, frame_lens, workspace,
                      workspace_bytes, stream);
}

extern "C" int ssak_w2v2_forward_hidden(ssak_w2v2* e, const float* input_values, const int32_t* lens, int B, int T,
                                        const uint8_t* spec_mask, const uint8_t* layer_keep , uint64_t seed,
                                        int training, void* hidden_bf16, int32_t* frame_lens, void* workspace,
                                        size_t workspace_bytes, void* stream) {
  SSAK_REQUIRE(e && hidden_bf16, "w2v2_forward_hidden: null pointer");
  if (e->cfg.exact)
    return forward_impl<float>(e, input_values, lens, B, T, spec_mask, layer_keep, seed, training, nullptr, hidden_bf16, frame_lens,
                               workspace, workspace_bytes, stream);
  return forward_impl<bf16>(e, input_values, lens, B, T, spec_mask, layer_keep, seed, training, nullptr, hidden_bf16, frame_lens,
                      workspace, workspace_bytes, stream);
}

template <typename AT>
int Call<AT>::bwd_zero_grads() {
  const long span = e->layer_span(), n_grad = e->n_grad();
  bool packed = true;
  for (int l = 1; l < c.num_layers; ++l) packed &= e->lp[l].wqkv == e->lp[l - 1].wqkv + span;
  const long w0 = e->lp[0].wqkv, w1 = e->lp[c.num_layers - 1].wqkv + span;
  if (!packed || w1 > n_grad) {
    SSAK_HIP(hipMemsetAsync(Gd, 0, (size_t)n_grad * sizeof(float), st));
  } else {
    if (w0 > 0) SSAK_HIP(hipMemsetAsync(Gd, 0, (size_t)w0 * sizeof(float), st));
    for (int l = 0; l < c.num_layers; ++l)
      if (!e->keep[l]) SSAK_HIP(hipMemsetAsync(Gd + e->lp[l].wqkv, 0, (size_t)span * sizeof(float), st));
    if (n_grad > w1) SSAK_HIP(hipMemsetAsync(Gd + w1, 0, (size_t)(n_grad - w1) * sizeof(float), st));
  }
  return SSAK_OK;
}

template <typename AT>
int Call<AT>::bwd_head(const float* dlogits, const void* dhidden, WgradQueue& wq) {
  AT* dlog = BF(p.dlog);
  if (dlogits) {
    if constexpr (EXACT)
      dlog = const_cast<float*>(dlogits);
    else
      TRY(k_cast_f32_bf16(dlogits, dlog, (long)M * V, st));
    TRY(k_colsum_t<AT>(dlog, V, M, V, Gd + e->p_lm_b, st, FP(p.lnpart), cs_floats));
  }
  if (!dlogits) TRY(wq.announce_in_order(e->p_lm_w, (long)V * H));
  gA = BF(p.dA);
  gB = nullptr;
  if (dhidden)
    SSAK_HIP(hipMemcpyAsync(gA, dhidden, (size_t)M * H * sizeof(AT), hipMemcpyDeviceToDevice, st));
  else {
    GemmX<EXACT> g(M, H, V);
    g.a(dlog, V).b(W + e->p_lm_w, H, true).c(gA, H);
    if (c.final_dropout > 0.f) g.drop(c.final_dropout, DS_FINAL, seed);
    TRY(g.run(st));
  }
  if (dlogits) {
    const AT* xl = (c.final_dropout > 0.f) ? BF(p.xf) : BF(e->xin[c.num_layers]);
    TRY(wq.push(GemmX<EXACT>(V, H, M).a(dlog, V, true).b(xl, H, true).c(Gd + e->p_lm_w, H, true), -1));
    TRY(wq.announce_after_last_product(e->p_lm_w, (long)V * H));
  }
  return SSAK_OK;
}

template <typename AT>
int Call<AT>::bwd_dropped_layer(int l, WgradQueue& wq, ReduceRing& red) {
  float* stl = FP(p.lb[l].st);
  float* ln_part = nullptr;
  TRY(red.get((size_t)LN_BWD_BLOCKS * 3 * H, &ln_part));
  const long nxt_w = next_ln_w(l), nxt_b = next_ln_b(l);
  TRY(wq.announce_in_order(e->lp[l].wqkv, e->layer_span()));
  if (!stable) return SSAK_OK;
  AT* dr = free_buf(gA, gB, Gres);
  TRY(k_layernorm_bwd_t<AT>(gA, gB, BF(e->hres[l]), stl + 2 * M, stl + 3 * M, P + nxt_w, Gres, dr, nullptr, Gd + nxt_w, Gd + nxt_b,
                      ln_part, M, H, none, none, st));
  Gres = dr;
  gA = BF(p.dB);
  gB = nullptr;
  SSAK_HIP(hipMemsetAsync(gA, 0, (size_t)M * H * sizeof(AT), st));
  return SSAK_OK;
}

template <typename AT>
int Call<AT>::bwd_layer(int l, WgradQueue& wq, ReduceRing& red) {
  const LayerP& L = e->lp[l];
  const LayerBuf& lb = p.lb[l];
  float* stl = FP(lb.st);
  float *ln_part = nullptr, *ln_part2 = nullptr, *ffn_part = nullptr, *qkv_part = nullptr;
  const size_t ln_part_floats = (size_t)LN_BWD_BLOCKS * 3 * H;
  TRY(red.get(ln_part_floats, &ln_part));
  const long nxt_w = next_ln_w(l), nxt_b = next_ln_b(l);
  TRY(red.get(ln_part_floats, &ln_part2));
  const size_t ffn_part_floats = (size_t)std::max(ssak_cdiv(M, 64), 64) * I;
  TRY(red.get(ffn_part_floats, &ffn_part));
  const size_t qkv_fused_floats = (p.fused_attn && !EXACT) ? k_attention_bwd_bias_floats(B, F, H) : 0;
  TRY(red.get(std::max((size_t)64 * 3 * H, qkv_fused_floats), &qkv_part));
  AT* dR = stable ? free_buf(gA, gB, Gres) : BF(p.dC);
  const int set = kept % WGRAD_SETS;
  ++kept;
  TRY(wq.reserve_set(set));
  AT* dY = BF(p.dYb[set]);
  AT* dY1 = BF(p.dY1b[set]);
  AT* dI = BF(p.dIb[set]);
  if (!stable) {
    TRY(k_layernorm_bwd_t<AT>(gA, gB, BF(lb.r2), stl + 2 * M, stl + 3 * M, P + L.ln2w, nullptr, dR, dY,
                        Gd + L.ln2w, Gd + L.ln2b, ln_part, M, H, DS(c.hidden_dropout, ds_hid2(l)), none, st, none, Gd + L.b2));
  } else {
    TRY(k_layernorm_bwd_t<AT>(gA, gB, BF(lb.r2), stl + 2 * M, stl + 3 * M, P + nxt_w, Gres, dR, dY, Gd + nxt_w,
                        Gd + nxt_b, ln_part, M, H, DS(c.hidden_dropout, ds_hid2(l)), none, st, none, Gd + L.b2));
  }
  const AT* dy2 = dY;
  TRY(wq.push(GemmX<EXACT>(H, I, M).a(dy2, H, true).b(BF(lb.f1), I, true).c(Gd + L.w2, I, true), set));
  TRY(GemmX<EXACT>(M, I, H).a(dy2, H).b_wt(EXACT ? nullptr : e->wt(l, 3), H, W + L.w2, I).c(dI, I)
          .epi(SSAK_EPI_MUL_AUX, BF(lb.f1pre))
          .drop(c.activation_dropout, ds_act(l), seed)
          .colsum(Gd + L.b1).run(st, ffn_part, ffn_part_floats * sizeof(float)));
  TRY(wq.push(GemmX<EXACT>(I, H, M).a(dI, I, true).b(BF(lb.x1), H, true).c(Gd + L.w1, H, true), set));
  AT* dX = BF(p.dB);
  TRY(GemmX<EXACT>(M, H, I).a(dI, I).b_wt(EXACT ? nullptr : e->wt(l, 2), I, W + L.w1, H).bfrag(e->wt(l, 2) ? nullptr : e->frag(l, 5)).c(dX, H).run(st));
  AT* dR1;
  if (!stable) {
    dR1 = BF(p.dA);
    TRY(k_layernorm_bwd_t<AT>(dR, dX, BF(lb.r1), stl, stl + M, P + L.ln1w, nullptr, dR1, dY1, Gd + L.ln1w,
                        Gd + L.ln1b, ln_part2, M, H, DS(c.hidden_dropout, ds_hid1(l)), none, st, none, Gd + L.bo));
  } else {
    dR1 = free_buf(dR, dX, nullptr);
    TRY(k_layernorm_bwd_t<AT>(dX, nullptr, BF(lb.r1), stl, stl + M, P + L.ln2w, dR, dR1, dY1, Gd + L.ln2w,
                        Gd + L.ln2b, ln_part2, M, H, DS(c.hidden_dropout, ds_hid1(l)), none, st, none, Gd + L.bo));
  }
  const AT* dy1 = dY1;
  TRY(wq.push(GemmX<EXACT>(H, H, M).a(dy1, H, true).b(BF(lb.ctx), H, true).c(Gd + L.wo, H, true), set));
  AT* dctx = free_buf(dR1, dX, nullptr);
// ... 17 lines not shown
    TRY(GemmX<EXACT>(F, hd, F).a(BF(p.dSb), Fp, true).b(qkv, 3 * H, true).c(dqkv + H, 3 * H).alpha(scale)
            .batch(B, nh, sp1, sp2, sq1, hd, sq1, hd).run(st));
  }
  TRY(wq.push(GemmX<EXACT>(3 * H, H, M).a(dqkv, 3 * H, true).b(BF(e->xin[l]), H, true).c(Gd + L.wqkv, H, true), set));
  if (!qkv_fused_floats) TRY(k_colsum_t<AT>(dqkv, 3 * H, M, 3 * H, Gd + L.bqkv, st, qkv_part, (size_t)64 * 3 * H));
  TRY(GemmX<EXACT>(M, H, 3 * H).a(dqkv, 3 * H).b_wt(EXACT ? nullptr : e->wt(l, 0), 3 * H, W + L.wqkv, H).bfrag(e->wt(l, 0) ? nullptr : e->frag(l, 3)).c(dX, H).run(st));
  TRY(wq.announce_after_last_product(L.wqkv, e->layer_span()));
  if ((kept & 1) == 0) TRY(red.flush());
  if (!stable) {
    gA = dR1;
    gB = dX;
  } else {
    gA = dX;
    gB = nullptr;
    Gres = dR1;
  }
  return SSAK_OK;
}

template <typename AT>
int Call<AT>::bwd_encoder_input(AT** dh1_out) {
  AT* dh1 = *dh1_out = free_buf(gA, gB, Gres);
  if (!stable) {
    TRY(k_layernorm_bwd_t<AT>(gA, gB, BF(p.h1), FP(p.stE), FP(p.stE) + M, P + e->p_eln_w, nullptr, dh1, nullptr, Gd + e->p_eln_w,
                        Gd + e->p_eln_b, FP(p.lnpart), M, H, none, DS(c.hidden_dropout, DS_ENCIN), st));
  } else {
    TRY(k_layernorm_bwd_t<AT>(gA, gB, BF(p.h1), FP(p.stE), FP(p.stE) + M, P + e->lp[0].ln1w, Gres, dh1, nullptr, Gd + e->lp[0].ln1w,
                        Gd + e->lp[0].ln1b, FP(p.lnpart), M, H, none, none, st, DS(c.hidden_dropout, DS_ENCIN)));
  }
  return SSAK_OK;
}

template <typename AT>
int Call<AT>::bwd_whisper_frontend(AT* dh1) {
  const int NM = c.num_mel_bins, Tin = p.Tin, RS1 = p.RS1, RS2 = p.RS2;
  AT* dpre2 = BF(p.dY);
  TRY(k_gelu_grad_mul_t<AT>(dh1, BF(p.wpre2), dpre2, (long)M * H, st));
  TRY(k_colsum_t<AT>(dpre2, H, M, H, Gd + e->p_c2b, st, FP(p.lnpart), cs_floats));
  TRY(k_copy_rows_padded_t<AT>(dpre2, BF(p.dpre2pad), B, F, RS2, H, st));
  TRY(GemmX<EXACT>(H, 3 * H, B * RS2).a(BF(p.dpre2pad), H, true).b(BF(p.h1pad), 2 * H, true).c(FP(p.dwr), 3 * H, true)
          .run_wgrad(st, slab, p.slab_bytes));
  TRY(k_conv_wgrad_unrearrange(FP(p.dwr), Gd + e->p_c2w, H, H, 3, st));
  TRY(GemmX<EXACT>(M, 3 * H, H).a(dpre2, H).b(e->conv_w[2], 3 * H, true).c(BF(p.dxcol), 3 * H).run(st));
  TRY(k_col2im_k3s2_t<AT>(BF(p.dxcol), BF(p.pre1), BF(p.dpre1pad), B, F, Tin, RS1, H, st));
  TRY(k_colsum_t<AT>(BF(p.dpre1pad), H, B * RS1, H, Gd + e->p_c1b, st, FP(p.lnpart), cs_floats));
  TRY(GemmX<EXACT>(H, 3 * NM, B * RS1).a(BF(p.dpre1pad), H, true).b(BF(p.melcl), NM, true).c(FP(p.dwr), 3 * NM, true)
          .run_wgrad(st, slab, p.slab_bytes));
  TRY(k_conv_wgrad_unrearrange(FP(p.dwr), Gd + e->p_c1w, H, NM, 3, st));
  for (int l = 0; l < c.num_layers; ++l)
    SSAK_HIP(hipMemsetAsync(Gd + e->lp[l].bqkv + H, 0, (size_t)H * sizeof(float), st));
  return SSAK_OK;
}

template <typename AT>
int Call<AT>::bwd_posconv_projection(AT* dh1) {
  AT* dpre = BF(p.dY);
  TRY(k_gelu_grad_mul_t<AT>(dh1, BF(p.pc_pre), dpre, (long)M * H, st));
  TRY(k_colsum_t<AT>(dpre, H, M, H, Gd + e->p_pc_b, st, FP(p.lnpart), cs_floats));
  TRY(k_posconv_pack_t<AT>(dpre, BF(p.pgdy), B, F, H, G, K, st));
  {
    const int lead = K / 2, RS = F + K;
    bool pcw_direct = false;
    if constexpr (!EXACT)
      pcw_direct = e->posconv_direct && e->pc_wf_frag != nullptr && k_posconv_wgrad_scratch_floats(H, G, K) * sizeof(float) <= p.slab_bytes;
    if (pcw_direct) {
      if constexpr (!EXACT)
        TRY(k_posconv_wgrad_direct(BF(p.pgx), BF(p.pgdy), p.pg_rows, (long)B * RS, lead, FP(p.dwf), reinterpret_cast<float*>(slab), H, G, K, st));
    } else {
      TRY(GemmX<EXACT>(K * cg, cg, B * RS)
              .a(BF(p.pgx), cg, true)
              .b(BF(p.pgdy) + (long)lead * cg, cg, true)
              .c(FP(p.dwf), cg, true)
              .batch(1, G, 0, p.pg_rows * cg, 0, p.pg_rows * cg, 0, (long)cg * K * cg)
              .run(st));
    }
    TRY(k_posconv_weight_bwd(FP(p.dwf), P + e->p_pc_g, P + e->p_pc_v, e->pc_norms, Gd + e->p_pc_g, Gd + e->p_pc_v, H, G, K, st));
    const int shift = 2 * (K / 2) - K + 1;
    bool pc_direct = false;
    if constexpr (!EXACT) pc_direct = e->posconv_direct && e->pc_wf_frag != nullptr;
    if (pc_direct) {
      if constexpr (!EXACT)
        TRY(k_posconv_direct(BF(p.pgdy), p.pg_rows, shift, e->pc_wb_frag, nullptr, BF(p.dB), nullptr, B, F, H, G, K, 0, st));
    } else {
      TRY(GemmX<EXACT>(F, cg, K * cg)
              .a(BF(p.pgdy) + (long)shift * cg, cg)
              .b(e->pc_wb, (long)K * cg)
              .c(BF(p.dB), H)
              .batch(B, G, (long)RS * cg, p.pg_rows * cg, 0, (long)cg * K * cg, (long)F * H, cg)
              .run(st));
    }
  }
  AT* dh0 = (dh1 == BF(p.dA)) ? BF(p.dC) : BF(p.dA);
  TRY(k_add_t<AT>(dh1, BF(p.dB), dh0, (long)M * H, st));
  TRY(k_specaug_bwd_t<AT>(dh0, e->spec_mask, flens, Gd + e->p_mse, B, F, H, st, FP(p.lnpart), cs_floats));
  const AT* dh0d = dh0;
  if (c.feat_proj_dropout > 0.f) {
    TRY(k_layernorm_fwd_t<AT>(dh0, nullptr, nullptr, nullptr, BF(p.scratchH), nullptr, nullptr, nullptr, M, H, 0.f,
                        DS(c.feat_proj_dropout, DS_FEATPROJ), none, st));
    dh0d = BF(p.scratchH);
  }
  TRY(GemmX<EXACT>(H, C, M).a(dh0d, H, true).b(BF(p.ln0), C, true).c(Gd + e->p_fp_w, C, true).run_wgrad(st, slab, p.slab_bytes));
  TRY(k_colsum_t<AT>(dh0d, H, M, H, Gd + e->p_fp_b, st, FP(p.lnpart), cs_floats));
  TRY(GemmX<EXACT>(M, C, H).a(dh0d, H).b(W + e->p_fp_w, C, true).c(BF(p.dln0), C).run(st));
  AT* dfeat = p.fe_train ? (((nc - 1) & 1) ? BF(p.fe_db) : BF(p.fe_da)) : BF(p.ln0);
  TRY(k_layernorm_bwd_t<AT>(BF(p.dln0), nullptr, BF(p.feat), FP(p.st0), FP(p.st0) + M, P + e->p_fpln_w, nullptr, dfeat, nullptr,
                      Gd + e->p_fpln_w, Gd + e->p_fpln_b, FP(p.lnpart), M, C, none, none, st));
  return SSAK_OK;
}

template <typename AT>
int Call<AT>::bwd_feature_encoder() {
  const bool ln_fe = c.feat_extract_norm == 1;
  for (int i = nc - 1; i >= 1; --i) {
    const int Ci = c.conv_dim[i - 1], Co = c.conv_dim[i], k = c.conv_kernel[i], s = c.conv_stride[i];
    const int Ti = p.Tl[i], Tp = p.Tl[i - 1];
    const AT* dact = (i & 1) ? BF(p.fe_db) : BF(p.fe_da);
    AT* dprev = ((i - 1) & 1) ? BF(p.fe_db) : BF(p.fe_da);
    const AT* act_prev = BF(p.act[i - 1]);
    if (ln_fe) {
      TRY(k_layernorm_bwd_t<AT>(dact, nullptr, BF(p.cpre[i]), FP(p.fe_st[i]), FP(p.fe_st[i]) + (size_t)B * Ti, P + e->p_cln_w[i], nullptr,
                          BF(p.fe_dp), BF(p.fe_dp), Gd + e->p_cln_w[i], Gd + e->p_cln_b[i], FP(p.lnpart), B * Ti, Co, none, none, st, none,
                          c.conv_bias ? Gd + e->p_conv_b[i] : nullptr, P + e->p_cln_b[i]));
    } else {
      TRY(k_gelu_grad_mul_t<AT>(dact, BF(p.cpre[i]), BF(p.fe_dp), (long)B * Ti * Co, st));
    }
    TRY(GemmX<EXACT>(Co, k * Ci, Ti).a(BF(p.fe_dp), Co, true).b(act_prev, (long)s * Ci, true).c(FP(p.fe_slab), (long)k * Ci, true)
            .batch(B, 1, (long)Ti * Co, 0, (long)Tp * Ci, 0, (long)Co * k * Ci, 0).run(st));
    TRY(k_sum_slabs(FP(p.fe_slab), B, (long)Co * k * Ci, FP(p.fe_dwr), st));
    TRY(k_conv_wgrad_unrearrange(FP(p.fe_dwr), Gd + e->p_conv_w[i], Co, Ci, k, st));
    TRY(GemmX<EXACT>(Ti, k * Ci, Co).a(BF(p.fe_dp), Co).b(e->conv_w[i], (long)k * Ci, true).c(BF(p.fe_dxcol), (long)k * Ci)
            .batch(B, 1, (long)Ti * Co, 0, 0, 0, (long)Ti * k * Ci, 0).run(st));
    TRY(k_col2im_t<AT>(BF(p.fe_dxcol), dprev, B, Tp, Ti, Ci, k, s, st));
  }
  if (ln_fe) {
    const int C0 = c.conv_dim[0], T0 = p.Tl[0];
    TRY(k_layernorm_bwd_t<AT>(BF(p.fe_da), nullptr, BF(p.cpre[0]), FP(p.fe_st[0]), FP(p.fe_st[0]) + (size_t)B * T0, P + e->p_cln_w[0], nullptr,
                        BF(p.fe_dp), BF(p.fe_dp), Gd + e->p_cln_w[0], Gd + e->p_cln_b[0], FP(p.lnpart), B * T0, C0, none, none, st, none,
                        c.conv_bias ? Gd + e->p_conv_b[0] : nullptr, P + e->p_cln_b[0]));
    TRY(k_conv0_wgrad_t<AT>(BF(p.fe_dp), e->last_input, Gd + e->p_conv_w[0], FP(p.fe_c0), B, p.T, T0, C0, c.conv_kernel[0],
                      c.conv_stride[0], st));
  } else {
    TRY(k_conv0_gn_gelu_bwd_t<AT>(e->last_input, P + e->p_conv_w[0], P + e->p_cln_w[0], P + e->p_cln_b[0], BF(p.fe_da),
                            (const double*)(ws + p.stats0), FP(p.fe_c0), Gd + e->p_conv_w[0], Gd + e->p_cln_w[0],
                            Gd + e->p_cln_b[0], B, p.T, p.Tl[0], c.conv_dim[0], st));
  }
  return SSAK_OK;
}

template <typename AT>
static int backward_impl(ssak_w2v2* e, const float* dlogits, const void* dhidden , void* workspace, size_t workspace_bytes,
                         void* stream) {
  SSAK_REQUIRE(e && (dlogits || dhidden) && workspace, "w2v2_backward: null pointer");
  SSAK_REQUIRE(e->cfg.adapter_attn_dim == 0,
               "w2v2_backward: a model with language adapters (adapter_attn_dim > 0) runs inference only: training is not implemented");
  if (!e->have_fwd || e->fwd_hidden != (dhidden != nullptr)) {
    ssak_set_error("w2v2_backward: no matching training-mode forward to differentiate");
    return SSAK_ERR_STATE;
  }
  EngineCall engine_call(e);
  SSAK_REQUIRE(e->G, "w2v2_backward: no gradient buffer bound");
  SSAK_REQUIRE(workspace_bytes >= e->plan.total, "w2v2_backward: workspace too small");
  Call<AT> k(e, workspace, stream, true);
  TRY(k.bwd_zero_grads());
  WgradQueue wq(e, k.st, k.slab, k.p.slab_bytes);
  TRY(k.bwd_head(dlogits, dhidden, wq));
  {
// ... 33 lines not shown
```

ssak_amd/hip.py:

```python
from __future__ import annotations

import ctypes as C
import os

import numpy as np
import torch

_DEFAULT_LIB = os.path.join(os.path.dirname(os.path.abspath(__file__)), "lib", "libssak_hip.so")
_LIB_PATH = os.environ.get("SSAK_HIP_LIB") or _DEFAULT_LIB
ABI_VERSION = 630


class GemmDesc(C.Structure):
    _fields_ = [("M", C.c_int), ("N", C.c_int), ("K", C.c_int), ("a_kmajor", C.c_int), ("b_kmajor", C.c_int),
                ("lda", C.c_long), ("ldb", C.c_long), ("ldc", C.c_long), ("nb1", C.c_int), ("nb2", C.c_int),
                ("sa1", C.c_long), ("sa2", C.c_long), ("sb1", C.c_long), ("sb2", C.c_long), ("sc1", C.c_long),
                ("sc2", C.c_long), ("alpha", C.c_float), ("epilogue", C.c_int), ("out_f32", C.c_int),
                ("accumulate", C.c_int), ("split_k", C.c_int), ("drop_p", C.c_float), ("drop_stream", C.c_uint32),
                ("drop_seed", C.c_uint64), ("bias_s2", C.c_long), ("pads_are_zero", C.c_int), ("colsum", C.c_int),
                ("dynamic_tiles", C.c_int), ("b_fragments", C.c_void_p), ("plan_tile", C.c_int)]


class W2V2Config(C.Structure):
    _fields_ = [("vocab_size", C.c_int), ("hidden_size", C.c_int), ("num_layers", C.c_int), ("num_heads", C.c_int),
                ("intermediate_size", C.c_int), ("num_conv_layers", C.c_int), ("conv_dim", C.c_int * 8),
                ("conv_kernel", C.c_int * 8), ("conv_stride", C.c_int * 8), ("conv_bias", C.c_int),
                ("feat_extract_norm", C.c_int), ("do_stable_layer_norm", C.c_int),
                ("num_conv_pos_embeddings", C.c_int), ("num_conv_pos_embedding_groups", C.c_int),
                ("layer_norm_eps", C.c_float), ("attention_dropout", C.c_float), ("hidden_dropout", C.c_float),
                ("activation_dropout", C.c_float), ("feat_proj_dropout", C.c_float), ("final_dropout", C.c_float),
                ("freeze_feature_encoder", C.c_int), ("arch", C.c_int), ("num_mel_bins", C.c_int),
                ("max_source_positions", C.c_int), ("exact", C.c_int), ("adapter_attn_dim", C.c_int)]


class ProfEntry(C.Structure):
    _fields_ = [("name", C.c_char * 112), ("launches", C.c_long), ("total_ms", C.c_double), ("total_flops", C.c_double),
                ("bound", C.c_int)]


class NgramLMDesc(C.Structure):
    _fields_ = [("order", C.c_int), ("n_words", C.c_int), ("bos", C.c_int), ("eos", C.c_int), ("unk", C.c_int),
                ("trie_cap", C.c_int), ("n_nodes", C.c_int), ("trie", C.c_void_p), ("node_word", C.c_void_p), ("uni", C.c_void_p),
                ("ng_keys", C.c_void_p * 6), ("ng_val", C.c_void_p * 6), ("ng_cap", C.c_int * 6)]


class LMBeamParams(C.Structure):
    _fields_ = [("beam_width", C.c_int), ("n_labels", C.c_int), ("blank", C.c_int), ("label_class", C.c_void_p),
                ("alpha", C.c_float), ("beta", C.c_float), ("beam_prune_logp", C.c_float), ("token_min_logp", C.c_float),
                ("unk_score_offset", C.c_float)]


class AudioBank(C.Structure):
    _fields_ = [("n", C.c_int), ("data", C.c_void_p), ("offset", C.c_void_p), ("length", C.c_void_p), ("offset_host", C.c_void_p),
                ("length_host", C.c_void_p)]


AUG_NONE, AUG_GAIN, AUG_NOISE_MIX, AUG_REVERB = -1, 0, 1, 2
(AUG_KIND, AUG_GAIN_DB, AUG_GAIN_LIN, AUG_SNR_DB, AUG_SNR_AMP, AUG_NOISE, AUG_NOISE_START, AUG_RIR, AUG_RIR_PEAK, AUG_RATE,
 AUG_OUT_LEN) = range(11)
AUG_NCOL = 11
AUG_FIR_MAX_TAPS, AUG_FIR_TILE = 255, 2048

GRAD_READY_FN = C.CFUNCTYPE(None, C.c_long, C.c_long, C.c_void_p)


def _load():
    if not os.path.exists(_LIB_PATH):
        raise ImportError(f"{_LIB_PATH} is missing: build it with `make` (or __graft_entry__.build()); "
                          "ssak_amd has no CPU fallback")
    lib = C.CDLL(_LIB_PATH)
    vp, i32, f32, sz = C.c_void_p, C.c_int, C.c_float, C.c_size_t
    sig = {
        "ssak_version": (i32, []),
        "ssak_last_error": (C.c_char_p, []),
        "ssak_wave_normalize_workspace_bytes": (sz, [i32, i32]),
        "ssak_wave_normalize": (i32, [vp, vp, i32, i32, vp, vp, vp, sz, vp]),
        "ssak_logmel_table_floats": (sz, []),
        "ssak_logmel_init_tables": (i32, [vp]),
        "ssak_logmel_workspace_bytes": (sz, [i32, i32]),
        "ssak_logmel_whisper": (i32, [vp, vp, i32, i32, i32, vp, vp, vp, i32, i32, vp, sz, vp]),
        "ssak_ctc_workspace_bytes": (sz, [i32, i32, i32, i32]),
        "ssak_ctc_loss_fwd_bwd": (i32, [vp, vp, vp, i32, i32, i32, i32, i32, i32, i32, f32, vp, vp, vp, vp, sz, vp]),
        "ssak_ctc_greedy_decode": (i32, [vp, vp, i32, i32, i32, i32, vp, vp, vp]),
        "ssak_augment_gain_noise_workspace_bytes": (sz, [i32, i32]),
        "ssak_augment_gain_noise": (i32, [vp, vp, vp, i32, i32, vp, vp, C.POINTER(AudioBank), vp, vp, sz, vp]),
        "ssak_augment_reverb_workspace_bytes": (sz, [i32, i32, i32]),
        "ssak_augment_reverb": (i32, [vp, vp, vp, i32, i32, vp, vp, C.POINTER(AudioBank), vp, vp, sz, vp]),
        "ssak_augment_time_stretch_workspace_bytes": (sz, [i32, i32, i32]),
        "ssak_augment_time_stretch": (i32, [vp, vp, vp, i32, i32, vp, vp, vp, vp, i32, vp, sz, vp]),
        "ssak_augment_fir_drop": (i32, [vp, i32, i32, vp, i32, vp, vp, vp, i32, vp, vp]),
        "ssak_ctc_lm_beam_workspace_bytes": (sz, [i32, i32, i32, i32]),
        "ssak_ctc_lm_beam_decode": (i32, [vp, vp, i32, i32, i32, C.POINTER(NgramLMDesc), C.POINTER(LMBeamParams), vp, vp, vp,
                                          vp, sz, vp]),
# ... 26 lines not shown
        "ssak_prof_collect": (i32, [vp, C.POINTER(ProfEntry), i32]),
        "ssak_attention_fwd": (i32, [vp, vp, vp, vp, i32, i32, i32, i32, f32, C.c_uint64, C.c_uint32, vp]),
        "ssak_attention_bwd": (i32, [vp, vp, vp, vp, vp, vp, vp, i32, i32, i32, i32, f32, C.c_uint64, C.c_uint32, i32, vp]),
        "ssak_attention_bwd_bias_workspace_bytes": (sz, [i32, i32, i32]),
        "ssak_attention_bwd_bias": (i32, [vp, vp, vp, vp, vp, vp, vp, vp, i32, i32, i32, i32, f32, C.c_uint64, C.c_uint32, vp, sz, vp]),
        "ssak_grad_sumsq": (i32, [vp, C.c_long, vp, vp, sz, vp]),
        "ssak_adamw_step": (i32, [vp, vp, vp, vp, vp, C.c_long, vp, f32, f32, f32, f32, f32, f32, f32, i32, vp]),
        "ssak_w2v2_create": (i32, [C.POINTER(W2V2Config), C.POINTER(vp)]),
        "ssak_w2v2_destroy": (None, [vp]),
        "ssak_w2v2_num_params": (C.c_long, [vp]),
        "ssak_w2v2_num_trainable": (C.c_long, [vp]),
        "ssak_w2v2_param_count": (i32, [vp]),
        "ssak_w2v2_param_info": (i32, [vp, i32, C.c_char_p, i32, C.POINTER(C.c_long), C.POINTER(C.c_long),
                                       C.POINTER(i32), C.POINTER(C.c_long)]),
        "ssak_w2v2_bind": (i32, [vp, vp, vp, vp]),
        "ssak_w2v2_sync_weights": (i32, [vp, i32, vp]),
        "ssak_w2v2_num_frames": (i32, [vp, i32]),
        "ssak_w2v2_workspace_bytes": (sz, [vp, i32, i32, i32]),
        "ssak_w2v2_forward": (i32, [vp, vp, vp, i32, i32, vp, vp, C.c_uint64, i32, vp, vp, vp, sz, vp]),
        "ssak_w2v2_backward": (i32, [vp, vp, vp, sz, vp]),
        "ssak_w2v2_set_grad_ready_callback": (i32, [vp, GRAD_READY_FN, vp]),
        "ssak_w2v2_set_param_event": (i32, [vp, vp, vp, vp]),
        "ssak_w2v2_set_option": (i32, [vp, i32, i32]),
        "ssak_w2v2_grad_ranges": (i32, [C.POINTER(W2V2Config), C.POINTER(C.c_long), C.POINTER(C.c_long), i32]),
        "ssak_w2v2_forward_hidden": (i32, [vp, vp, vp, i32, i32, vp, vp, C.c_uint64, i32, vp, vp, vp, sz, vp]),
        "ssak_w2v2_backward_hidden": (i32, [vp, vp, vp, sz, vp]),
        "ssak_grad_sumsq_add": (i32, [vp, C.c_long, vp, vp, sz, vp]),
        "ssak_utt_norm_workspace_bytes": (sz, [i32]),
        "ssak_utt_norm_fwd": (i32, [vp, vp, i32, C.c_long, i32, f32, vp, vp, sz, vp]),
        "ssak_utt_norm_bwd": (i32, [vp, vp, vp, i32, C.c_long, i32, vp, vp, sz, vp]),
        "ssak_batchnorm_workspace_bytes": (sz, [i32]),
        "ssak_batchnorm_act_fwd": (i32, [vp, vp, i32, i32, vp, vp, vp, vp, f32, f32, i32, f32, f32, C.c_uint64, C.c_uint32, vp, vp,
                                         vp, vp, sz, vp]),
        "ssak_batchnorm_act_bwd": (i32, [vp, vp, vp, i32, i32, vp, vp, vp, vp, f32, f32, C.c_uint64, C.c_uint32, vp, vp, vp, vp,
                                         vp, sz, vp]),
        "ssak_batchnorm_stats": (i32, [vp, i32, i32, vp, vp, sz, vp]),
        "ssak_adadelta_step": (i32, [vp, vp, vp, vp, vp, C.c_long, vp, f32, f32, f32, f32, f32, f32, vp]),
        "ssak_cast_f32_bf16": (i32, [vp, vp, C.c_long, vp]),
        "ssak_cast_bf16_f32": (i32, [vp, vp, C.c_long, vp]),
        "ssak_colsum_workspace_bytes": (sz, [i32]),
        "ssak_colsum_bf16": (i32, [vp, C.c_long, i32, i32, vp, vp, sz, vp]),
        "ssak_comm_unique_id": (i32, [vp]),
        "ssak_comm_create": (i32, [C.POINTER(vp), i32, i32, vp]),
        "ssak_allreduce": (i32, [vp, vp, C.c_long, C.c_long, i32, vp]),
        "ssak_comm_destroy": (i32, [vp]),
        "ssak_pool_fwd": (i32, [vp, vp, vp, i32, i32, i32, i32, i32, vp, vp, vp]),
        "ssak_pool_bwd": (i32, [vp, vp, vp, vp, i32, i32, i32, i32, i32, vp, vp]),
        "ssak_cls_head_fwd": (i32, [vp, vp, vp, vp, vp, i32, i32, i32, f32, C.c_uint64, i32, vp, vp, vp]),
        "ssak_cls_head_bwd_workspace_bytes": (sz, [i32, i32, i32]),
        "ssak_cls_head_bwd": (i32, [vp, vp, vp, vp, vp, i32, i32, i32, f32, C.c_uint64, i32, vp, vp, vp, vp, vp, vp, sz, vp]),
        "ssak_cls_softmax_ce": (i32, [vp, vp, vp, i32, i32, f32, vp, vp, vp, vp]),
        "ssak_dec_embed": (i32, [vp, vp, vp, vp, i32, i32, i32, i32, i32, i32, vp, vp]),
        "ssak_dec_attention_fwd": (i32, [vp, C.c_long, vp, C.c_long, vp, C.c_long, i32, vp, vp, i32, i32, i32, i32, i32, i32, vp, vp]),
        "ssak_token_logprobs": (i32, [vp, i32, i32, i32, C.c_long, vp, vp, vp, vp, i32, vp, vp, vp, vp, vp]),
        "ssak_dec_attention_step_workspace_bytes": (sz, [i32, i32, i32]),
        "ssak_dec_attention_step": (i32, [vp, C.c_long, vp, C.c_long, C.c_long, vp, C.c_long, C.c_long, i32, vp, i32, i32, i32, i32, vp, sz, vp, vp]),
        "ssak_dec_greedy_step": (i32, [vp, C.c_long, i32, i32, vp, vp, i32, vp, vp, i32, i32, i32, i32, i32, vp, vp, vp, vp, C.c_long, i32, vp, vp]),
        "ssak_dec_timestamp_step": (i32, [vp, C.c_long, i32, i32, vp, vp, i32, i32, i32, i32, vp, vp, i32, i32, i32, i32, i32, vp, vp, vp, vp, C.c_long,
                                          i32, vp, vp, vp]),
        "ssak_dec_beam_topk": (i32, [vp, C.c_long, i32, i32, i32, vp, vp, i32, i32, i32, i32, i32, i32, vp, C.c_long, i32, vp, vp, i32, vp, vp, vp]),
        "ssak_dec_beam_select": (i32, [vp, vp, i32, i32, i32, i32, vp, vp, vp, vp, C.c_long, i32, vp, i32, vp, vp, vp, vp, vp, vp, vp, vp, vp, i32,
                                       i32, i32, i32, i32, vp, vp]),
        "ssak_dec_kv_reorder": (i32, [vp, vp, i32, i32, i32, i32, i32, C.c_long, C.c_long, C.c_long, i32, i32, vp]),
        "ssak_dec_attention_step_grouped": (i32, [vp, C.c_long, vp, C.c_long, C.c_long, vp, C.c_long, C.c_long, i32, vp, i32, i32, i32, i32, i32, vp,
                                                  sz, vp, vp]),
        "ssak_layernorm_fwd": (i32, [vp, vp, vp, vp, vp, vp, i32, i32, f32, i32, vp]),
        "ssak_debug_dropout_mask": (i32, [C.c_uint64, C.c_uint32, f32, C.c_long, i32, vp, C.POINTER(f32), vp]),
        "ssak_debug_attention_dropout_mask": (i32, [C.c_uint64, C.c_uint32, f32, i32, i32, i32, vp, vp]),
        "ssak_debug_layernorm_fwd": (i32, [vp, vp, vp, vp, vp, vp, vp, vp, i32, i32, f32, C.c_uint64, C.c_uint32, f32, C.c_uint32,
                                            f32, C.c_uint32, f32, i32, i32, vp]),
        "ssak_debug_layernorm_bwd_workspace_bytes": (sz, [i32]),
        "ssak_debug_layernorm_bwd": (i32, [vp, vp, vp, vp, vp, vp, vp, vp, vp, vp, vp, vp, vp, i32, i32, C.c_uint64, C.c_uint32, f32,
                                            C.c_uint32, f32, C.c_uint32, f32, i32, i32, vp, sz, vp]),
        "ssak_debug_softmax_fwd": (i32, [vp, vp, vp, vp, i32, i32, i32, i32, C.c_uint64, C.c_uint32, f32, i32, vp]),
        "ssak_debug_softmax_bwd": (i32, [vp, vp, vp, i32, i32, i32, C.c_uint64, C.c_uint32, f32, i32, vp]),
        "ssak_debug_gelu": (i32, [vp, C.c_long, vp, vp, i32, vp]),
        "ssak_test_attn_adapter_fwd": (i32, [vp, vp, vp, vp, vp, vp, vp, vp, vp, vp, vp, vp, vp, vp, i32, i32, i32, f32, f32, i32, vp]),
        "ssak_debug_posconv_prepare": (i32, [vp, vp, vp, vp, vp, i32, i32, i32, i32, vp]),
        "ssak_debug_posconv_pack": (i32, [vp, vp, i32, i32, i32, i32, i32, i32, vp]),
        "ssak_debug_posconv_workspace_bytes": (sz, [i32, i32, i32, i32, i32]),
        "ssak_debug_posconv_direct": (i32, [vp, vp, vp, vp, vp, i32, i32, i32, i32, i32, i32, i32, vp, sz, vp]),
        "ssak_debug_posconv_wgrad": (i32, [vp, vp, vp, i32, i32, i32, i32, i32, vp, sz, vp]),
        "ssak_debug_posconv_weight_bwd": (i32, [vp, vp, vp, vp, vp, vp, i32, i32, i32, vp]),
        "ssak_debug_conv0_bwd_workspace_bytes": (sz, [i32, i32, i32]),
        "ssak_debug_conv0_bwd": (i32, [vp, vp, vp, vp, vp, vp, vp, vp, vp, i32, i32, i32, i32, vp, sz, vp]),
        "ssak_debug_conv0_wgrad_workspace_bytes": (sz, [i32, i32, i32]),
        "ssak_debug_conv0_wgrad": (i32, [vp, vp, vp, i32, i32, i32, i32, i32, i32, vp, sz, vp]),
        "ssak_debug_conv0_bias": (i32, [vp, vp, vp, vp, i32, i32, i32, i32, vp]),
        "ssak_debug_col2im": (i32, [vp, vp, i32, i32, i32, i32, i32, i32, i32, vp]),
        "ssak_debug_sum_slabs": (i32, [vp, i32, C.c_long, vp, vp]),
        "ssak_debug_conv_weight_rearrange": (i32, [vp, vp, i32, i32, i32, i32, vp]),
        "ssak_debug_conv_wgrad_unrearrange": (i32, [vp, vp, i32, i32, i32, vp]),
        "ssak_debug_col2im_k3s2": (i32, [vp, vp, vp, i32, i32, i32, i32, i32, i32, vp]),
        "ssak_debug_mel_to_cl": (i32, [vp, vp, i32, i32, i32, i32, i32, i32, vp]),
        "ssak_debug_add_rowvec": (i32, [vp, vp, vp, i32, i32, i32, i32, vp]),
        "ssak_debug_copy_rows_padded": (i32, [vp, vp, i32, i32, i32, i32, i32, vp]),
    }
    lib.ssak_version.restype = i32
    got = lib.ssak_version()
    if got != ABI_VERSION:
        raise ImportError(f"{_LIB_PATH} reports ABI {got}, this binding is written for {ABI_VERSION}: rebuild with `make`"
                          + (" (SSAK_HIP_LIB must name a build of the same ABI)" if os.environ.get("SSAK_HIP_LIB") else ""))
    for name, (res, args) in sig.items():
        fn = getattr(lib, name)
        fn.restype, fn.argtypes = res, args
    return lib


lib = _load()
SSAK_OK, SSAK_ERR_INVALID, SSAK_ERR_LAUNCH, SSAK_ERR_STATE = 0, -1, -2, -3
EPI_NONE, EPI_GELU, EPI_MUL_GELU_GRAD, EPI_GELU_SAVE_GRAD, EPI_MUL_AUX = 0, 1, 2, 3, 4
REDUCTION = {"sum": 0, "mean": 1}


def check(rc: int):
    if rc == SSAK_OK:
        return
    msg = lib.ssak_last_error().decode()
    if rc == SSAK_ERR_INVALID:
        raise ValueError(msg)
    if rc == SSAK_ERR_STATE:
        raise RuntimeError(msg)
    raise RuntimeError(f"libssak_hip status {rc}: {msg}")


def ptr(t):
    return None if t is None else C.c_void_p(t.data_ptr())


def stream():
    return C.c_void_p(torch.cuda.current_stream().cuda_stream)


def _ws(nbytes: int, device):
    return torch.empty(max(int(nbytes), 16), dtype=torch.uint8, device=device)


def wave_normalize(x: torch.Tensor, lens: torch.Tensor | None = None, return_mask: bool = False):
    assert x.is_cuda and x.dtype == torch.float32 and x.dim() == 2 and x.is_contiguous()
    B, T = x.shape
    out = torch.empty_like(x)
    mask = torch.empty((B, T), dtype=torch.int32, device=x.device) if return_mask else None
    if lens is not None:
        lens = lens.to(device=x.device, dtype=torch.int32).contiguous()
    ws = _ws(lib.ssak_wave_normalize_workspace_bytes(B, T), x.device)
    check(lib.ssak_wave_normalize(ptr(x), ptr(lens), B, T, ptr(out), ptr(mask), ptr(ws), ws.numel(), stream()))
    return (out, mask) if return_mask else out


_LOGMEL_TABLES = {}


def logmel_tables(device):
    key = str(device)
    if key not in _LOGMEL_TABLES:
        t = torch.empty(lib.ssak_logmel_table_floats(), dtype=torch.float32, device=device)
        check(lib.ssak_logmel_init_tables(ptr(t)))
        _LOGMEL_TABLES[key] = t
    return _LOGMEL_TABLES[key]


def logmel_whisper(wav: torch.Tensor, lens: torch.Tensor | None = None, n_samples: int = 480000,
                   channels_last: torch.Tensor | None = None, cl_lead: int = 0, want_mel: bool = True):
    assert wav.is_cuda and wav.dtype == torch.float32 and wav.dim() == 2 and wav.is_contiguous()
    B, T = wav.shape
    if lens is not None:
# ... 585 lines not shown
def debug_layernorm_bwd(g1, g2, r, mean, rstd, gamma, g_res, dr, dy, dgamma, dbeta, dy_colsum=None, post_gelu_beta=None, *, seed=0,
                        pre=(0, 0.0), mid=(0, 0.0), post=(0, 0.0), queued=False, workspace=None):
    M, Cc = r.shape
    nbytes = lib.ssak_debug_layernorm_bwd_workspace_bytes(Cc)
    ws = workspace if workspace is not None else _ws(nbytes, r.device)
    check(lib.ssak_debug_layernorm_bwd(ptr(g1), ptr(g2), ptr(r), ptr(mean), ptr(rstd), ptr(gamma), ptr(g_res), ptr(dr), ptr(dy),
                                       ptr(dgamma), ptr(dbeta), ptr(dy_colsum), ptr(post_gelu_beta), M, Cc, seed, pre[0], float(pre[1]),
                                       mid[0], float(mid[1]), post[0], float(post[1]), int(bool(queued)), _row_dtype(r), ptr(ws),
                                       ws.numel(), stream()))


def debug_softmax_fwd(S, P, Pd, klens, cols: int, rows_per_batch: int = 1, *, seed=0, site=0, p=0.0):
    rows, ld = S.shape
    check(lib.ssak_debug_softmax_fwd(ptr(S), ptr(P), ptr(Pd), ptr(klens), rows, cols, ld, rows_per_batch, seed, site, float(p),
                                     _row_dtype(S), stream()))


def debug_softmax_bwd(dPd, P, dS, cols: int, *, seed=0, site=0, p=0.0):
    rows, ld = P.shape
    check(lib.ssak_debug_softmax_bwd(ptr(dPd), ptr(P), ptr(dS), rows, cols, ld, seed, site, float(p), _row_dtype(P), stream()))


def debug_gelu(x: torch.Tensor, dtype: torch.dtype):
    assert x.is_cuda and x.dtype == torch.float32 and x.is_contiguous()
    y, d = torch.empty_like(x), torch.empty_like(x)
    check(lib.ssak_debug_gelu(ptr(x), x.numel(), ptr(y), ptr(d), 0 if dtype == torch.bfloat16 else 1, stream()))
    return y, d


def test_attn_adapter_fwd(y, res, ln_g, ln_b, w1, b1, w2, b2, next_g, next_b, r_out, out, mean=None, rstd=None, *, eps_adapter=1e-5,
                          eps_next=1e-5):
    M, H = res.shape
    A = w1.shape[0]
    dt = _row_dtype(res)
    assert all(t is None or t.dtype == res.dtype for t in (y, w1, w2, r_out, out)), "activations and W1 / W2 share one storage type"
    check(lib.ssak_test_attn_adapter_fwd(ptr(y), ptr(res), ptr(ln_g), ptr(ln_b), ptr(w1), ptr(b1), ptr(w2), ptr(b2), ptr(next_g),
                                         ptr(next_b), ptr(r_out), ptr(out), ptr(mean), ptr(rstd), M, H, A, float(eps_adapter),
                                         float(eps_next), dt, stream()))


test_attn_adapter_fwd.__test__ = False


def debug_posconv_prepare(g: torch.Tensor, v: torch.Tensor, G: int, dtype: torch.dtype = torch.bfloat16):
    H, cg, K = v.shape
    nan = float("nan")
    wf = torch.full((H, K, cg), nan, dtype=dtype, device=v.device)
    wb = torch.full((G, cg, K, cg), nan, dtype=dtype, device=v.device)
    norms = torch.full(((2 + H) * K,), nan, dtype=torch.float32, device=v.device)
    check(lib.ssak_debug_posconv_prepare(ptr(g), ptr(v), ptr(wf), ptr(wb), ptr(norms), H, G, K, _row_dtype(wf), stream()))
    return wf, wb, norms


def debug_posconv_pack(h: torch.Tensor, B: int, F: int, G: int, K: int):
    H = h.shape[1]
    pg = torch.full((G, K // 2 + B * (F + K) + K, H // G), float("nan"), dtype=h.dtype, device=h.device)
    check(lib.ssak_debug_posconv_pack(ptr(h), ptr(pg), B, F, H, G, K, _row_dtype(h), stream()))
    return pg


def debug_posconv_workspace(B: int, F: int, H: int, G: int, K: int, device):
    nbytes = lib.ssak_debug_posconv_workspace_bytes(B, F, H, G, K)
    return torch.full((max(int(nbytes), 16),), 0xFF, dtype=torch.uint8, device=device)


def debug_posconv_direct(h, w, bias, out, pre, B: int, F: int, G: int, K: int, *, row0=0, gelu=False, workspace=None):
    H = h.shape[1]
    ws = workspace if workspace is not None else debug_posconv_workspace(B, F, H, G, K, h.device)
    check(lib.ssak_debug_posconv_direct(ptr(h), ptr(w), ptr(bias), ptr(out), ptr(pre), B, F, H, G, K, int(row0), int(bool(gelu)),
                                        ptr(ws), ws.numel(), stream()))


def debug_posconv_wgrad(h, dpre, dwf, B: int, F: int, G: int, K: int, *, workspace=None):
    H = h.shape[1]
    ws = workspace if workspace is not None else debug_posconv_workspace(B, F, H, G, K, h.device)
    check(lib.ssak_debug_posconv_wgrad(ptr(h), ptr(dpre), ptr(dwf), B, F, H, G, K, ptr(ws), ws.numel(), stream()))


def debug_posconv_weight_bwd(dwf, g, v, norms, dg, dv, G: int):
    H, cg, K = v.shape
    check(lib.ssak_debug_posconv_weight_bwd(ptr(dwf), ptr(g), ptr(v), ptr(norms), ptr(dg), ptr(dv), H, G, K, stream()))


def debug_conv0_bwd_workspace(B: int, T: int, C_: int, device):
    nbytes = lib.ssak_debug_conv0_bwd_workspace_bytes(B, T, C_)
    return torch.full((max(int(nbytes), 16),), 0xFF, dtype=torch.uint8, device=device)


def debug_conv0_bwd(x, w, gamma, beta, dy, sums, dw, dgamma, dbeta, *, workspace=None):
    B, T = x.shape
    Cc = w.shape[0]
    ws = workspace if workspace is not None else debug_conv0_bwd_workspace(B, T, Cc, x.device)
    check(lib.ssak_debug_conv0_bwd(ptr(x), ptr(w), ptr(gamma), ptr(beta), ptr(dy), ptr(sums), ptr(dw), ptr(dgamma), ptr(dbeta), B, T, Cc,
                                   _row_dtype(dy), ptr(ws), ws.numel(), stream()))


def debug_conv0_wgrad(d, x, dw, stride: int, *, workspace=None):
    B, T = x.shape
    Cc, ksize = dw.shape
    nbytes = lib.ssak_debug_conv0_wgrad_workspace_bytes(B, Cc, ksize)
    ws = workspace if workspace is not None else torch.full((max(int(nbytes), 16),), 0xFF, dtype=torch.uint8, device=x.device)
    check(lib.ssak_debug_conv0_wgrad(ptr(d), ptr(x), ptr(dw), B, T, Cc, ksize, int(stride), _row_dtype(d), ptr(ws), ws.numel(), stream()))


def debug_conv0_bias(x, w, bias, out):
    B, T = x.shape
    check(lib.ssak_debug_conv0_bias(ptr(x), ptr(w), ptr(bias), ptr(out), B, T, w.shape[0], _row_dtype(out), stream()))


def debug_col2im(dxcol, dx, k: int, s: int):
    B, Tout, kk, Cc = dxcol.shape
    assert kk == k and dx.shape[0] == B and dx.shape[2] == Cc
    check(lib.ssak_debug_col2im(ptr(dxcol), ptr(dx), B, dx.shape[1], Tout, Cc, k, s, _row_dtype(dx), stream()))


def debug_sum_slabs(slabs, out):
    nb, n = slabs.shape
    check(lib.ssak_debug_sum_slabs(ptr(slabs), nb, n, ptr(out), stream()))


def debug_conv_weight_rearrange(w, out):
    Co, Ci, k = w.shape
    check(lib.ssak_debug_conv_weight_rearrange(ptr(w), ptr(out), Co, Ci, k, _row_dtype(out), stream()))


def debug_conv_wgrad_unrearrange(dwr, g):
    Co, Ci, k = g.shape
    check(lib.ssak_debug_conv_wgrad_unrearrange(ptr(dwr), ptr(g), Co, Ci, k, stream()))


def debug_col2im_k3s2(dxcol, pre, out, Tin: int):
    B, F, _, H = dxcol.shape
    check(lib.ssak_debug_col2im_k3s2(ptr(dxcol), ptr(pre), ptr(out), B, F, Tin, out.shape[1], H, _row_dtype(out), stream()))


def debug_mel_to_cl(mel, cl, RS: int, lead: int):
    B, Cc, T = mel.shape
    check(lib.ssak_debug_mel_to_cl(ptr(mel), ptr(cl), B, Cc, T, RS, lead, _row_dtype(cl), stream()))


def debug_add_rowvec(x, pos, out):
    B, F, H = x.shape
    check(lib.ssak_debug_add_rowvec(ptr(x), ptr(pos), ptr(out), B, F, H, _row_dtype(x), stream()))


def debug_copy_rows_padded(src, dst):
    B, F, H = src.shape
    check(lib.ssak_debug_copy_rows_padded(ptr(src), ptr(dst), B, F, dst.shape[1], H, _row_dtype(src), stream()))
```

Measured before the change: 2224 utterances/sec.

## Add fused skinny CTC head kernels and direct frag posconv weight prep

Adds dedicated MFMA kernels for the CTC vocabulary head (V<=64). The forward kernel fuses final dropout, the bf16 dropped-activation write and bias into the logits GEMM. The backward kernel fuses the dlogits cast, the bias-gradient column sum and the input-gradient GEMM with the dropout mask. Positional-conv weight preparation now writes fragment-layout weights directly and builds the plain bf16 weights lazily, only when the GEMM fallback needs them. This aims to cut launches and extra passes over small-N GEMMs, at the cost of new custom code paths with double-precision partial reductions.

After: 2229 utterances/sec (median of 3 runs). Within noise of the previous version (+0.2%).

```diff
diff --git a/include/ssak_hip.h b/include/ssak_hip.h
--- a/include/ssak_hip.h
+++ b/include/ssak_hip.h
@@ -383,6 +383,16 @@
 int ssak_debug_posconv_weight_bwd(const float* dwf, const float* g, const float* v, float* norms, float* dg, float* dv, int H, int G,
                                   int K, void* stream);
 
+int ssak_debug_posconv_prepare_frag(const float* g, const float* v, void* wf_frag, void* wb_frag, float* norms, int H, int G, int K,
+                                    void* stream);
+int ssak_debug_posconv_frag(const void* w, void* wfrag, int H, int G, int K, void* stream);
+int ssak_debug_colsum(const void* x, int M, int N, float* out, void* workspace, size_t workspace_bytes, void* stream);
+size_t ssak_debug_head_workspace_bytes(int M, int V);
+int ssak_debug_head_fwd(const void* x, const void* w, const float* bias, void* xf, float* logits, int M, int H, int V, uint64_t seed,
+                        uint32_t site, float p, void* stream);
+int ssak_debug_head_bwd(const float* dlogits, const void* w, void* dlog, float* dbias, void* ga, int M, int H, int V, uint64_t seed,
+                        uint32_t site, float p, void* workspace, size_t workspace_bytes, void* stream);
+
 size_t ssak_debug_conv0_bwd_workspace_bytes(int B, int T, int C);
 int ssak_debug_conv0_bwd(const float* x, const float* w, const float* gamma, const float* beta, const void* dy, const double* sums,
                          float* dw, float* dgamma, float* dbeta, int B, int T, int C, int dtype, void* workspace, size_t workspace_bytes,
diff --git a/ssak_amd/csrc/api.cpp b/ssak_amd/csrc/api.cpp
--- a/ssak_amd/csrc/api.cpp
+++ b/ssak_amd/csrc/api.cpp
@@ -17,7 +17,7 @@
   va_end(ap);
 }
 
-extern "C" int ssak_version(void) { return 630; }
+extern "C" int ssak_version(void) { return 640; }
 extern "C" const char* ssak_last_error(void) { return g_err; }
 
 #include <atomic>
diff --git a/ssak_amd/csrc/conv_frontend.hip b/ssak_amd/csrc/conv_frontend.hip
--- a/ssak_amd/csrc/conv_frontend.hip
+++ b/ssak_amd/csrc/conv_frontend.hip
@@ -754,17 +754,24 @@
   return SSAK_OK;
 }
 
+int k_posconv_norms(const float* v, float* norms, int H, int G, int K, hipStream_t st) {
+  SSAK_REQUIRE(K <= 1024 && H % G == 0 && ((H / G) & 7) == 0, "posconv: K=%d <= 1024 and (H/G)=%d %% 8 == 0 required", K, H / G);
+  const int cg = H / G;
+  float* partial = norms + 2 * K;
+  posconv_colnorm_kernel<<<H, ((K + 63) / 64) * 64, 0, st>>>(v, nullptr, H / cg, K, cg, partial);
+  SSAK_LAUNCH_CHECK();
+  posconv_colnorm_finalize_kernel<<<ssak_cdiv(K, 64), 1024, 0, st>>>(partial, H, K, norms);
+  SSAK_LAUNCH_CHECK();
+  return SSAK_OK;
+}
+
 template <typename OT>
 int k_posconv_prepare_t(const float* g, const float* v, OT* w_fwd, OT* w_bwd, float* norms, int H, int G, int K,
                         hipStream_t st) {
   SSAK_REQUIRE(K <= 1024 && H % G == 0 && ((H / G) & 7) == 0, "posconv: K=%d <= 1024 and (H/G)=%d %% 8 == 0 required", K, H / G);
   const int cg = H / G;
-  float* partial = norms + 2 * K;
   ProfScope prof_scope(PROF_POSCONV_W, (double)H * cg * K * 8.0, st);
-  posconv_colnorm_kernel<<<H, ((K + 63) / 64) * 64, 0, st>>>(v, nullptr, H / cg, K, cg, partial);
-  SSAK_LAUNCH_CHECK();
-  posconv_colnorm_finalize_kernel<<<ssak_cdiv(K, 64), 1024, 0, st>>>(partial, H, K, norms);
-  SSAK_LAUNCH_CHECK();
+  if (int rc = k_posconv_norms(v, norms, H, G, K, st)) return rc;
   SSAK_REQUIRE((size_t)cg * (K + 1) * sizeof(float) <= 64 * 1024, "posconv: (H/G) x K slab does not fit in LDS");
   posconv_materialize_kernel<OT><<<2 * H, 256, (size_t)cg * (K + 1) * sizeof(float), st>>>(g, v, norms, w_fwd, w_bwd, H, cg, K);
   SSAK_LAUNCH_CHECK();
diff --git a/ssak_amd/csrc/head.hip b/ssak_amd/csrc/head.hip
--- /dev/null
+++ b/ssak_amd/csrc/head.hip
@@ -0,0 +1,322 @@
+#include <algorithm>
+
+#include "common.h"
+#include "kernels.h"
+
+namespace {
+
+SSAK_DEFINE_DROP_TABLE
+
+struct HeadParams {
+  const bf16* x;
+  const bf16* w;
+  const float* bias;
+  bf16* xf;
+  float* logits;
+  const float* dlogits;
+  bf16* dlog;
+  double* part;
+  bf16* ga;
+  int M, H, V;
+  uint64_t seed;
+  uint32_t stream, thresh;
+  float scale;
+};
+
+template <int NJ>
+__global__ __launch_bounds__(256) void head_fwd_kernel(const HeadParams p) {
+  extern __shared__ __attribute__((aligned(16))) char hf_lds[];
+  const int lane = threadIdx.x & 63, wave = threadIdx.x >> 6;
+  const int lc = lane & 15, g4 = lane >> 4;
+  const int m = (blockIdx.x * 4 + wave) * 16 + lc;
+  const bool rowok = m < p.M;
+  const size_t xo = (size_t)(rowok ? m : 0) * p.H + 8 * g4;
+  constexpr int U = 8;
+  Chunk8<bf16> cur[U], nxt[U];
+  auto load = [&](Chunk8<bf16> (&dst)[U], int k0) {
+#pragma unroll
+    for (int u = 0; u < U; ++u) {
+      dst[u] = Chunk8<bf16>{};
+      if (rowok && k0 + 32 * u < p.H) dst[u] = ld8<bf16>(p.x + xo + k0 + 32 * u);
+    }
+  };
+  load(cur, 0);
+  const int pitch = (p.H + 8) * 2, hc = p.H >> 3;
+  for (int i = threadIdx.x; i < 16 * NJ * hc; i += 256) {
+    const int v = i / hc, c = i % hc;
+    uint4 raw = make_uint4(0u, 0u, 0u, 0u);
+    if (v < p.V) raw = *reinterpret_cast<const uint4*>(p.w + (size_t)v * p.H + c * 8);
+    *reinterpret_cast<uint4*>(hf_lds + v * pitch + c * 16) = raw;
+  }
+  uint32_t* cml = reinterpret_cast<uint32_t*>(hf_lds + 16 * NJ * pitch);
+  if (p.thresh)
+    for (int i = threadIdx.x; i < p.H; i += 256) cml[i] = g_drop_colmul.v[i];
+  __syncthreads();
+  const uint32_t rk = p.thresh ? drop_rowkey(p.seed, p.stream, (uint64_t)m) : 1u;
+  const uint32_t thi = p.thresh << 16;
+  f32x4 acc[NJ];
+#pragma unroll
+  for (int j = 0; j < NJ; ++j) acc[j] = (f32x4){0.f, 0.f, 0.f, 0.f};
+  const char* wl = hf_lds + lc * pitch + 16 * g4;
+  auto step = [&](int k0, Chunk8<bf16> a) {
+    if (p.thresh) {
+      float f[8];
+      chunk_to_f(a, f);
+      const uint32_t* cmp = cml + k0 + 8 * g4;
+      const uint4 c0 = *reinterpret_cast<const uint4*>(cmp), c1 = *reinterpret_cast<const uint4*>(cmp + 4);
+      const uint32_t cm[8] = {c0.x, c0.y, c0.z, c0.w, c1.x, c1.y, c1.z, c1.w};
+#pragma unroll
+      for (int k = 0; k < 8; ++k) f[k] = drop_keep(rk, cm[k], thi) ? f[k] * p.scale : 0.f;
+      a = f_to_chunk8<bf16>(f);
+    }
+    if (p.xf && rowok) st8<bf16>(p.xf + xo + k0, a);
+    const bf16x8 fa = __builtin_bit_cast(bf16x8, a.q);
+#pragma unroll
+    for (int j = 0; j < NJ; ++j)
+      acc[j] = __builtin_amdgcn_mfma_f32_16x16x32_bf16(*reinterpret_cast<const bf16x8*>(wl + 16 * j * pitch + k0 * 2), fa, acc[j], 0, 0, 0);
+  };
+  for (int k0 = 0; k0 < p.H; k0 += 32 * U) {
+    load(nxt, k0 + 32 * U);
+#pragma unroll
+    for (int u = 0; u < U; ++u)
+      if (k0 + 32 * u < p.H) step(k0 + 32 * u, cur[u]);
+#pragma unroll
+    for (int u = 0; u < U; ++u) cur[u] = nxt[u];
+  }
+  if (!rowok) return;
+#pragma unroll
+  for (int j = 0; j < NJ; ++j) {
+    const int v0 = 16 * j + 4 * g4;
+    if (v0 < p.V) {
+      const float4 b = *reinterpret_cast<const float4*>(p.bias + v0);
+      const float4 o = make_float4(acc[j][0] + b.x, acc[j][1] + b.y, acc[j][2] + b.z, acc[j][3] + b.w);
+      *reinterpret_cast<float4*>(p.logits + (size_t)m * p.V + v0) = o;
+    }
+  }
+}
+
+template <int VP>
+__global__ __launch_bounds__(256) void head_bwd_kernel(const HeadParams p) {
+  constexpr int KS = VP / 32, PITCH = (VP + 8) * 2;
+  extern __shared__ __attribute__((aligned(16))) char hd_lds[];
+  const int lane = threadIdx.x & 63, wave = threadIdx.x >> 6;
+  const int lc = lane & 15, g4 = lane >> 4;
+  const int hc = p.H >> 3;
+  for (int i = threadIdx.x; i < VP * hc; i += 256) {
+    const int v = i % VP, c = i / VP;
+    uint4 raw = make_uint4(0u, 0u, 0u, 0u);
+    if (v < p.V) raw = *reinterpret_cast<const uint4*>(p.w + (size_t)v * p.H + c * 8);
+    const uint32_t wd[4] = {raw.x, raw.y, raw.z, raw.w};
+#pragma unroll
+    for (int e = 0; e < 8; ++e)
+      *reinterpret_cast<uint16_t*>(hd_lds + (c * 8 + e) * PITCH + v * 2) = (uint16_t)(wd[e >> 1] >> (16 * (e & 1)));
+  }
+  uint32_t* cml = reinterpret_cast<uint32_t*>(hd_lds + (size_t)p.H * PITCH);
+  if (p.thresh)
+    for (int i = threadIdx.x; i < p.H; i += 256) cml[i] = g_drop_colmul.v[i];
+  __syncthreads();
+  const uint32_t thi = p.thresh << 16;
+  double cs[KS][8];
+#pragma unroll
+  for (int ks = 0; ks < KS; ++ks)
+#pragma unroll
+    for (int e = 0; e < 8; ++e) cs[ks][e] = 0.0;
+  const int ntiles = (p.M + 15) / 16;
+  for (int tile = blockIdx.x * 4 + wave; tile < ntiles; tile += gridDim.x * 4) {
+    const int m = tile * 16 + lc;
+    const bool rowok = m < p.M;
+    const uint32_t rk = p.thresh ? drop_rowkey(p.seed, p.stream, (uint64_t)m) : 1u;
+    bf16x8 fa[KS];
+#pragma unroll
+    for (int ks = 0; ks < KS; ++ks) {
+      const int v0 = 32 * ks + 8 * g4;
+      float f[8] = {0.f, 0.f, 0.f, 0.f, 0.f, 0.f, 0.f, 0.f};
+      const bool in = rowok && v0 < p.V;
+      if (in) {
+        const float* src = p.dlogits + (size_t)m * p.V + v0;
+        *reinterpret_cast<float4*>(f) = *reinterpret_cast<const float4*>(src);
+        *reinterpret_cast<float4*>(f + 4) = *reinterpret_cast<const float4*>(src + 4);
+      }
+      const Chunk8<bf16> q = f_to_chunk8<bf16>(f);
+      if (in) st8<bf16>(p.dlog + (size_t)m * p.V + v0, q);
+      chunk_to_f(q, f);
+#pragma unroll
+      for (int e = 0; e < 8; ++e) cs[ks][e] += (double)f[e];
+      fa[ks] = __builtin_bit_cast(bf16x8, q.q);
+    }
+    bf16* orow = p.ga + (size_t)(rowok ? m : 0) * p.H + 4 * g4;
+    const int nj = p.H / 16;
+    for (int j0 = 0; j0 < nj; j0 += 4) {
+      f32x4 acc[4];
+#pragma unroll
+      for (int jj = 0; jj < 4; ++jj) {
+        acc[jj] = (f32x4){0.f, 0.f, 0.f, 0.f};
+        const int j = min(j0 + jj, nj - 1);
+        const char* wrow = hd_lds + (16 * j + lc) * PITCH + 16 * g4;
+#pragma unroll
+        for (int ks = 0; ks < KS; ++ks)
+          acc[jj] = __builtin_amdgcn_mfma_f32_16x16x32_bf16(*reinterpret_cast<const bf16x8*>(wrow + 64 * ks), fa[ks], acc[jj], 0, 0, 0);
+      }
+#pragma unroll
+      for (int jj = 0; jj < 4; ++jj) {
+        const int j = j0 + jj;
+        if (j < nj) {
+          if (p.thresh) {
+            const uint4 t = *reinterpret_cast<const uint4*>(cml + 16 * j + 4 * g4);
+            const uint32_t cm[4] = {t.x, t.y, t.z, t.w};
+#pragma unroll
+            for (int r = 0; r < 4; ++r) acc[jj][r] = drop_keep(rk, cm[r], thi) ? acc[jj][r] * p.scale : 0.f;
+          }
+          if (rowok) {
+            const bf16x4 o = {(bf16)acc[jj][0], (bf16)acc[jj][1], (bf16)acc[jj][2], (bf16)acc[jj][3]};
+            *reinterpret_cast<bf16x4*>(orow + 16 * j) = o;
+          }
+        }
+      }
+    }
+  }
+#pragma unroll
+  for (int ks = 0; ks < KS; ++ks)
+#pragma unroll
+    for (int e = 0; e < 8; ++e) {
+      double s = cs[ks][e];
+      s += __shfl_xor(s, 1);
+      s += __shfl_xor(s, 2);
+      s += __shfl_xor(s, 4);
+      s += __shfl_xor(s, 8);
+      cs[ks][e] = s;
+    }
+  __syncthreads();
+  double* red = reinterpret_cast<double*>(hd_lds);
+  if (lc == 0) {
+#pragma unroll
+    for (int ks = 0; ks < KS; ++ks)
+#pragma unroll
+      for (int e = 0; e < 8; ++e) red[wave * VP + 32 * ks + 8 * g4 + e] = cs[ks][e];
+  }
+  __syncthreads();
+  if ((int)threadIdx.x < p.V)
+    p.part[(size_t)blockIdx.x * p.V + threadIdx.x] =
+        ((red[threadIdx.x] + red[VP + threadIdx.x]) + red[2 * VP + threadIdx.x]) + red[3 * VP + threadIdx.x];
+}
+
+__global__ __launch_bounds__(1024) void head_bias_finalize_kernel(const double* __restrict__ part, int slots, int V, float* __restrict__ out) {
+  __shared__ double red[16][65];
+  const int v = threadIdx.x & 63, ry = threadIdx.x >> 6;
+  double s = 0.0;
+  if (v < V)
+    for (int k = ry; k < slots; k += 16) s += part[(size_t)k * V + v];
+  red[ry][v] = s;
+  __syncthreads();
+  if (ry == 0 && v < V) {
+    double t = 0.0;
+#pragma unroll
+    for (int r = 0; r < 16; ++r) t += red[r][v];
+    out[v] += (float)t;
+  }
+}
+
+uint32_t hd_thresh(float p) { return p <= 0.f ? 0u : (uint32_t)fminf(65535.f, roundf(p * 65536.f)); }
+float hd_scale(float p) { return p <= 0.f ? 1.f : 1.f / (1.f - (float)hd_thresh(p) / 65536.f); }
+constexpr int HD_BWD_MAX_BLOCKS = 512;
+int hd_bwd_blocks(int M) { return std::min(HD_BWD_MAX_BLOCKS, ssak_cdiv(ssak_cdiv(M, 16), 4)); }
+size_t hd_bwd_lds(int H, int V) { return (size_t)H * ((V <= 32 ? 32 : 64) + 8) * 2 + (size_t)H * 4; }
+size_t hd_fwd_lds(int H, int V) { return (size_t)16 * ssak_cdiv(V, 16) * (H + 8) * 2 + (size_t)H * 4; }
+
+}
+
+bool k_head_supported(int H, int V) {
+  return V >= 8 && V <= 64 && (V & 7) == 0 && H >= 32 && (H & 31) == 0 && H <= DROP_TABLE_N && hd_bwd_lds(H, V) <= 150 * 1024 &&
+         hd_fwd_lds(H, V) <= 150 * 1024;
+}
+size_t k_head_bwd_scratch_floats(int M, int V) { return (size_t)hd_bwd_blocks(M) * V * 2 + 2; }
+
+int k_head_fwd(const bf16* x, const bf16* w, const float* bias, bf16* xf, float* logits, int M, int H, int V, const DropSpec& drop,
+               hipStream_t st) {
+  SSAK_REQUIRE(k_head_supported(H, V) && M > 0, "head_fwd: M=%d H=%d V=%d not built", M, H, V);
+  SSAK_REQUIRE(xf || drop.p <= 0.f, "head_fwd: the dropped activation needs its output buffer");
+  HeadParams p{};
+  p.x = x, p.w = w, p.bias = bias, p.xf = xf, p.logits = logits;
+  p.M = M, p.H = H, p.V = V;
+  p.seed = drop.seed, p.stream = drop.stream, p.thresh = hd_thresh(drop.p), p.scale = hd_scale(drop.p);
+  ProfScope prof_scope(PROF_ROWWISE, (double)M * H * 2.0 * (xf ? 2 : 1) + (double)M * V * 4.0, st);
+  const int grid = ssak_cdiv(ssak_cdiv(M, 16), 4);
+  const size_t lds = hd_fwd_lds(H, V);
+  static bool attr_done = false;
+  if (!attr_done) {
+    SSAK_HIP(hipFuncSetAttribute((const void*)head_fwd_kernel<1>, hipFuncAttributeMaxDynamicSharedMemorySize, 160 * 1024));
+    SSAK_HIP(hipFuncSetAttribute((const void*)head_fwd_kernel<2>, hipFuncAttributeMaxDynamicSharedMemorySize, 160 * 1024));
+    SSAK_HIP(hipFuncSetAttribute((const void*)head_fwd_kernel<3>, hipFuncAttributeMaxDynamicSharedMemorySize, 160 * 1024));
+    SSAK_HIP(hipFuncSetAttribute((const void*)head_fwd_kernel<4>, hipFuncAttributeMaxDynamicSharedMemorySize, 160 * 1024));
+    attr_done = true;
+  }
+  switch (ssak_cdiv(V, 16)) {
+    case 1: head_fwd_kernel<1><<<grid, 256, lds, st>>>(p); break;
+    case 2: head_fwd_kernel<2><<<grid, 256, lds, st>>>(p); break;
+    case 3: head_fwd_kernel<3><<<grid, 256, lds, st>>>(p); break;
+    default: head_fwd_kernel<4><<<grid, 256, lds, st>>>(p); break;
+  }
+  SSAK_LAUNCH_CHECK();
+  return SSAK_OK;
+}
+
+int k_head_bwd(const float* dlogits, const bf16* w, bf16* dlog, float* dbias, bf16* ga, float* scratch, size_t scratch_floats, int M,
+               int H, int V, const DropSpec& drop, hipStream_t st) {
+  SSAK_REQUIRE(k_head_supported(H, V) && M > 0, "head_bwd: M=%d H=%d V=%d not built", M, H, V);
+  const int grid = hd_bwd_blocks(M);
+  SSAK_REQUIRE(scratch && scratch_floats >= k_head_bwd_scratch_floats(M, V), "head_bwd: scratch too small");
+  double* part = reinterpret_cast<double*>(((uintptr_t)scratch + 7) & ~(uintptr_t)7);
+  HeadParams p{};
+  p.w = w, p.dlogits = dlogits, p.dlog = dlog, p.part = part, p.ga = ga;
+  p.M = M, p.H = H, p.V = V;
+  p.seed = drop.seed, p.stream = drop.stream, p.thresh = hd_thresh(drop.p), p.scale = hd_scale(drop.p);
+  const size_t lds = hd_bwd_lds(H, V);
+  ProfScope prof_scope(PROF_ROWWISE, (double)M * H * 2.0 + (double)M * V * 6.0, st);
+  if (V <= 32) {
+    static bool attr32 = false;
+    if (!attr32) {
+      SSAK_HIP(hipFuncSetAttribute((const void*)head_bwd_kernel<32>, hipFuncAttributeMaxDynamicSharedMemorySize, 160 * 1024));
+      attr32 = true;
+    }
+    head_bwd_kernel<32><<<grid, 256, lds, st>>>(p);
+  } else {
+    static bool attr64 = false;
+    if (!attr64) {
+      SSAK_HIP(hipFuncSetAttribute((const void*)head_bwd_kernel<64>, hipFuncAttributeMaxDynamicSharedMemorySize, 160 * 1024));
+      attr64 = true;
+    }
+    head_bwd_kernel<64><<<grid, 256, lds, st>>>(p);
+  }
+  SSAK_LAUNCH_CHECK();
+  head_bias_finalize_kernel<<<1, 1024, 0, st>>>(part, grid, V, dbias);
+  SSAK_LAUNCH_CHECK();
+  return SSAK_OK;
+}
+
+extern "C" size_t ssak_debug_head_workspace_bytes(int M, int V) { return (M > 0 && V > 0) ? k_head_bwd_scratch_floats(M, V) * sizeof(float) : 0; }
+
+extern "C" int ssak_debug_head_fwd(const void* x, const void* w, const float* bias, void* xf, float* logits, int M, int H, int V,
+                                   uint64_t seed, uint32_t site, float p, void* stream) {
+  SSAK_REQUIRE(x && w && bias && logits && (xf || p <= 0.f), "debug_head_fwd: null pointer");
+  SSAK_REQUIRE(M > 0 && k_head_supported(H, V), "debug_head_fwd: M=%d H=%d V=%d not built", M, H, V);
+  DropSpec d;
+  d.seed = seed, d.stream = site, d.p = p;
+  return k_head_fwd((const bf16*)x, (const bf16*)w, bias, (bf16*)xf, logits, M, H, V, d, (hipStream_t)stream);
+}
+
+extern "C" int ssak_debug_head_bwd(const float* dlogits, const void* w, void* dlog, float* dbias, void* ga, int M, int H, int V,
+                                   uint64_t seed, uint32_t site, float p, void* workspace, size_t workspace_bytes, void* stream) {
+  SSAK_REQUIRE(dlogits && w && dlog && dbias && ga && workspace, "debug_head_bwd: null pointer");
+  SSAK_REQUIRE(M > 0 && k_head_supported(H, V), "debug_head_bwd: M=%d H=%d V=%d not built", M, H, V);
+  DropSpec d;
+  d.seed = seed, d.stream = site, d.p = p;
+  return k_head_bwd(dlogits, (const bf16*)w, (bf16*)dlog, dbias, (bf16*)ga, (float*)workspace, workspace_bytes / sizeof(float), M, H, V,
+                    d, (hipStream_t)stream);
+}
+
+extern "C" int ssak_debug_colsum(const void* x, int M, int N, float* out, void* workspace, size_t workspace_bytes, void* stream) {
+  SSAK_REQUIRE(x && out && workspace && M > 0 && N > 0 && (N & 7) == 0, "debug_colsum: null pointer or bad shape M=%d N=%d", M, N);
+  const size_t need = (size_t)std::min(64, ssak_cdiv(M, 32)) * N;
+  SSAK_REQUIRE(workspace_bytes >= need * sizeof(float), "debug_colsum: workspace too small");
+  return k_colsum_t<bf16>((const bf16*)x, N, M, N, out, (hipStream_t)stream, (float*)workspace, need);
+}
diff --git a/ssak_amd/csrc/kernels.h b/ssak_amd/csrc/kernels.h
--- a/ssak_amd/csrc/kernels.h
+++ b/ssak_amd/csrc/kernels.h
@@ -122,6 +122,7 @@
 template <typename T>
 int k_posconv_prepare_t(const float* g, const float* v, T* w_fwd, T* w_bwd, float* norms, int H, int G, int K,
                         hipStream_t st);
+int k_posconv_norms(const float* v, float* norms, int H, int G, int K, hipStream_t st);
 int k_posconv_weight_bwd(const float* dw, const float* g, const float* v, const float* norms, float* dg, float* dv,
                          int H, int G, int K, hipStream_t st);
 template <typename T>
@@ -144,12 +145,21 @@
 
 bool k_posconv_direct_supported(int H, int G, int K);
 int k_posconv_frag_weights(const bf16* w, bf16* wfrag, int H, int G, int K, hipStream_t st);
+int k_posconv_prepare_frag(const float* g, const float* v, bf16* wf_frag, bf16* wb_frag, float* norms, int H, int G, int K,
+                           hipStream_t st);
 int k_posconv_direct(const bf16* x, long rows_per_group, int row0, const bf16* w, const float* bias, bf16* out, bf16* pre, int B, int F,
                      int H, int G, int K, int gelu, hipStream_t st);
 
 size_t k_posconv_wgrad_scratch_floats(int H, int G, int K);
 int k_posconv_wgrad_direct(const bf16* x, const bf16* dy, long rows_per_group, long rows, int lead, float* dwf, float* scratch, int H, int G,
                            int K, hipStream_t st);
+
+bool k_head_supported(int H, int V);
+size_t k_head_bwd_scratch_floats(int M, int V);
+int k_head_fwd(const bf16* x, const bf16* w, const float* bias, bf16* xf, float* logits, int M, int H, int V, const DropSpec& drop,
+               hipStream_t st);
+int k_head_bwd(const float* dlogits, const bf16* w, bf16* dlog, float* dbias, bf16* ga, float* scratch, size_t scratch_floats, int M,
+               int H, int V, const DropSpec& drop, hipStream_t st);
 
 template <typename T_>
 int k_mel_to_cl_t(const float* mel, T_* cl, int B, int C, int T, int RS, int lead, hipStream_t st);
diff --git a/ssak_amd/csrc/posconv.hip b/ssak_amd/csrc/posconv.hip
--- a/ssak_amd/csrc/posconv.hip
+++ b/ssak_amd/csrc/posconv.hip
@@ -182,6 +182,87 @@
   return SSAK_OK;
 }
 
+namespace {
+
+constexpr int PF_KN = 32;
+template <int CG, int VW>
+__global__ __launch_bounds__(256) void posconv_prepare_frag_kernel(const float* __restrict__ g, const float* __restrict__ v,
+                                                                   const float* __restrict__ nsq, bf16* __restrict__ wf_frag,
+                                                                   bf16* __restrict__ wb_frag, int G, int K) {
+  using G_ = PcGeom<CG>;
+  constexpr int TP = G_::TP, KK = G_::KK, NJ = G_::NJ;
+  extern __shared__ __attribute__((aligned(16))) char pf_lds[];
+  bf16* tile = reinterpret_cast<bf16*>(pf_lds);
+  const int nkb = (K + PF_KN - 1) / PF_KN;
+  int id = blockIdx.x;
+  const int kb = id % nkb;
+  id /= nkb;
+  const int j = id % NJ;
+  id /= NJ;
+  const int grp = id % G;
+  const bool back = id / G != 0;
+  const int k0 = kb * PF_KN, nk = min(PF_KN, K - k0);
+  const int per = nk / VW;
+  for (int t = threadIdx.x; t < 16 * CG * per; t += 256) {
+    const int pi = t / per, kl = (t % per) * VW;
+    int r16, cc;
+    long src;
+    if (!back) {
+      r16 = pi / CG, cc = pi % CG;
+      src = ((long)(grp * CG + 16 * j + r16) * CG + cc) * K;
+    } else {
+      cc = pi / 16, r16 = pi % 16;
+      src = ((long)(grp * CG + cc) * CG + 16 * j + r16) * K;
+    }
+    float x[VW];
+    if constexpr (VW == 4)
+      *reinterpret_cast<float4*>(x) = *reinterpret_cast<const float4*>(v + src + k0 + kl);
+    else
+      x[0] = v[src + k0 + kl];
+#pragma unroll
+    for (int u = 0; u < VW; ++u) {
+      const int k = k0 + kl + u;
+      tile[((r16 * PF_KN) + kl + u) * CG + cc] = (bf16)(g[k] * x[u] * rsqrtf(nsq[k]));
+    }
+  }
+  __syncthreads();
+  const int nsteps = K / TP;
+  const int s0 = (back ? K - k0 - nk : k0) / TP, ns = nk / TP;
+  bf16* dst = back ? wb_frag : wf_frag;
+  for (int t = threadIdx.x; t < ns * KK * 64; t += 256) {
+    const int lane = t & 63, kk = (t >> 6) % KK, sl = (t >> 6) / KK;
+    const int lc = lane & 15, g4 = lane >> 4;
+    const int rem = 32 * kk + 8 * g4, tp = rem / CG, c = rem % CG;
+    const int ot = (s0 + sl) * TP + tp;
+    const int kl = back ? (K - 1 - ot) - k0 : ot - k0;
+    const long chunk = ((((long)grp * nsteps + s0 + sl) * NJ + j) * KK + kk) * 64 + lane;
+    *reinterpret_cast<uint4*>(dst + chunk * 8) = *reinterpret_cast<const uint4*>(tile + ((lc * PF_KN) + kl) * CG + c);
+  }
+}
+
+template <int CG>
+int launch_prepare_frag(const float* g, const float* v, const float* nsq, bf16* wf_frag, bf16* wb_frag, int G, int K, hipStream_t st) {
+  constexpr size_t lds = (size_t)16 * PF_KN * CG * sizeof(bf16);
+  const int grid = 2 * G * PcGeom<CG>::NJ * ((K + PF_KN - 1) / PF_KN);
+  if ((K & 3) == 0 && ((uintptr_t)v & 15) == 0)
+    posconv_prepare_frag_kernel<CG, 4><<<grid, 256, lds, st>>>(g, v, nsq, wf_frag, wb_frag, G, K);
+  else
+    posconv_prepare_frag_kernel<CG, 1><<<grid, 256, lds, st>>>(g, v, nsq, wf_frag, wb_frag, G, K);
+  SSAK_LAUNCH_CHECK();
+  return SSAK_OK;
+}
+
+}
+
+int k_posconv_prepare_frag(const float* g, const float* v, bf16* wf_frag, bf16* wb_frag, float* norms, int H, int G, int K,
+                           hipStream_t st) {
+  SSAK_REQUIRE(k_posconv_direct_supported(H, G, K), "posconv_prepare_frag: H=%d G=%d K=%d not built", H, G, K);
+  ProfScope prof_scope(PROF_POSCONV_W, (double)H * (H / G) * K * 8.0, st);
+  if (int rc = k_posconv_norms(v, norms, H, G, K, st)) return rc;
+  return H / G == 48 ? launch_prepare_frag<48>(g, v, norms, wf_frag, wb_frag, G, K, st)
+                     : launch_prepare_frag<64>(g, v, norms, wf_frag, wb_frag, G, K, st);
+}
+
 int k_posconv_direct(const bf16* x, long rows_per_group, int row0, const bf16* w, const float* bias, bf16* out, bf16* pre, int B, int F,
                      int H, int G, int K, int gelu, hipStream_t st) {
   SSAK_REQUIRE(k_posconv_direct_supported(H, G, K), "posconv_direct: H=%d G=%d K=%d not built", H, G, K);
@@ -454,3 +535,16 @@
   if (rc != SSAK_OK) return rc;
   return k_posconv_wgrad_direct(px, pdy, ws.rows_per_group, (long)B * (F + K), K / 2, dwf, (float*)(base + ws.scratch), H, G, K, st);
 }
+
+extern "C" int ssak_debug_posconv_prepare_frag(const float* g, const float* v, void* wf_frag, void* wb_frag, float* norms, int H, int G,
+                                               int K, void* stream) {
+  SSAK_REQUIRE(g && v && wf_frag && wb_frag && norms, "debug_posconv_prepare_frag: null pointer");
+  SSAK_REQUIRE(k_posconv_direct_supported(H, G, K), "debug_posconv_prepare_frag: H=%d G=%d K=%d not built", H, G, K);
+  return k_posconv_prepare_frag(g, v, (bf16*)wf_frag, (bf16*)wb_frag, norms, H, G, K, (hipStream_t)stream);
+}
+
+extern "C" int ssak_debug_posconv_frag(const void* w, void* wfrag, int H, int G, int K, void* stream) {
+  SSAK_REQUIRE(w && wfrag, "debug_posconv_frag: null pointer");
+  SSAK_REQUIRE(k_posconv_direct_supported(H, G, K), "debug_posconv_frag: H=%d G=%d K=%d not built", H, G, K);
+  return k_posconv_frag_weights((const bf16*)w, (bf16*)wfrag, H, G, K, (hipStream_t)stream);
+}
diff --git a/ssak_amd/csrc/w2v2_engine.hip b/ssak_amd/csrc/w2v2_engine.hip
--- a/ssak_amd/csrc/w2v2_engine.hip
+++ b/ssak_amd/csrc/w2v2_engine.hip
@@ -75,6 +75,7 @@
   void* pc_wb = nullptr;
   bf16* pc_wf_frag = nullptr;
   bf16* pc_wb_frag = nullptr;
+  bool pc_plain_valid = false;
   float* pc_norms = nullptr;
   Plan plan;
   bool have_fwd = false;
@@ -885,7 +886,12 @@
   if (c.exact)
     TRY(k_posconv_prepare_t<float>(e->P + e->p_pc_g, e->P + e->p_pc_v, (float*)e->pc_wf, (float*)e->pc_wb, e->pc_norms, c.hidden_size,
                                    c.num_conv_pos_embedding_groups, c.num_conv_pos_embeddings, st));
-  else {
+  else if (e->pc_wf_frag && e->posconv_direct) {
+    TRY(k_posconv_prepare_frag(e->P + e->p_pc_g, e->P + e->p_pc_v, e->pc_wf_frag, e->pc_wb_frag, e->pc_norms, c.hidden_size,
+                               c.num_conv_pos_embedding_groups, c.num_conv_pos_embeddings, st));
+    e->pc_plain_valid = false;
+    return SSAK_OK;
+  } else {
     TRY(k_posconv_prepare_t<bf16>(e->P + e->p_pc_g, e->P + e->p_pc_v, (bf16*)e->pc_wf, (bf16*)e->pc_wb, e->pc_norms, c.hidden_size,
                                   c.num_conv_pos_embedding_groups, c.num_conv_pos_embeddings, st));
     if (e->pc_wf_frag) {
@@ -893,6 +899,16 @@
       TRY(k_posconv_frag_weights((const bf16*)e->pc_wb, e->pc_wb_frag, c.hidden_size, c.num_conv_pos_embedding_groups, c.num_conv_pos_embeddings, st));
     }
   }
+  e->pc_plain_valid = true;
+  return SSAK_OK;
+}
+
+static int posconv_plain_weights(ssak_w2v2* e, hipStream_t st) {
+  if (e->pc_plain_valid) return SSAK_OK;
+  const ssak_w2v2_config& c = e->cfg;
+  TRY(k_posconv_prepare_t<bf16>(e->P + e->p_pc_g, e->P + e->p_pc_v, (bf16*)e->pc_wf, (bf16*)e->pc_wb, e->pc_norms, c.hidden_size,
+                                c.num_conv_pos_embedding_groups, c.num_conv_pos_embeddings, st));
+  e->pc_plain_valid = true;
   return SSAK_OK;
 }
 
@@ -1083,6 +1099,7 @@
     if constexpr (!EXACT)
       TRY(k_posconv_direct(BF(p.pgx), p.pg_rows, 0, e->pc_wf_frag, P + e->p_pc_b, BF(p.pc), BF(p.pc_pre), B, F, H, G, K, 1, st));
   } else {
+    if constexpr (!EXACT) TRY(posconv_plain_weights(e, st));
     TRY(GemmX<EXACT>(F, cg, K * cg)
             .a(BF(p.pgx), cg)
             .b(e->pc_wf, (long)K * cg)
@@ -1174,6 +1191,15 @@
     return SSAK_OK;
   }
   e->fwd_hidden = false;
+  if constexpr (!EXACT) {
+    if (k_head_supported(H, V)) {
+      const bool drop = tr && c.final_dropout > 0.f;
+      TRY(k_head_fwd(xl, W + e->p_lm_w, P + e->p_lm_b, drop ? BF(p.xf) : nullptr, logits, M, H, V,
+                     drop ? DS(c.final_dropout, DS_FINAL) : none, st));
+      e->have_fwd = tr;
+      return SSAK_OK;
+    }
+  }
   if (tr && c.final_dropout > 0.f) {
     TRY(k_layernorm_fwd_t<AT>(xl, nullptr, nullptr, nullptr, BF(p.xf), nullptr, nullptr, nullptr, M, H, 0.f,
                         DS(c.final_dropout, DS_FINAL), none, st));
@@ -1270,7 +1296,15 @@
 template <typename AT>
 int Call<AT>::bwd_head(const float* dlogits, const void* dhidden, WgradQueue& wq) {
   AT* dlog = BF(p.dlog);
-  if (dlogits) {
+  bool skinny = false;
+  if constexpr (!EXACT) skinny = dlogits && !dhidden && k_head_supported(H, V) && cs_floats >= k_head_bwd_scratch_floats(M, V);
+  if (skinny) {
+    gA = BF(p.dA);
+    gB = nullptr;
+    if constexpr (!EXACT)
+      TRY(k_head_bwd(dlogits, W + e->p_lm_w, dlog, Gd + e->p_lm_b, gA, FP(p.lnpart), cs_floats, M, H, V,
+                     DS(c.final_dropout, DS_FINAL), st));
+  } else if (dlogits) {
     if constexpr (EXACT)
       dlog = const_cast<float*>(dlogits);
     else
@@ -1280,7 +1314,8 @@
   if (!dlogits) TRY(wq.announce_in_order(e->p_lm_w, (long)V * H));
   gA = BF(p.dA);
   gB = nullptr;
-  if (dhidden)
+  if (skinny) {
+  } else if (dhidden)
     SSAK_HIP(hipMemcpyAsync(gA, dhidden, (size_t)M * H * sizeof(AT), hipMemcpyDeviceToDevice, st));
   else {
     GemmX<EXACT> g(M, H, V);
@@ -1464,6 +1499,7 @@
       if constexpr (!EXACT)
         TRY(k_posconv_direct(BF(p.pgdy), p.pg_rows, shift, e->pc_wb_frag, nullptr, BF(p.dB), nullptr, B, F, H, G, K, 0, st));
     } else {
+      if constexpr (!EXACT) TRY(posconv_plain_weights(e, st));
       TRY(GemmX<EXACT>(F, cg, K * cg)
               .a(BF(p.pgdy) + (long)shift * cg, cg)
               .b(e->pc_wb, (long)K * cg)
diff --git a/ssak_amd/hip.py b/ssak_amd/hip.py
--- a/ssak_amd/hip.py
+++ b/ssak_amd/hip.py
@@ -8,7 +8,7 @@
 
 _DEFAULT_LIB = os.path.join(os.path.dirname(os.path.abspath(__file__)), "lib", "libssak_hip.so")
 _LIB_PATH = os.environ.get("SSAK_HIP_LIB") or _DEFAULT_LIB
-ABI_VERSION = 630
+ABI_VERSION = 640
 
 
 class GemmDesc(C.Structure):
@@ -201,6 +201,12 @@
         "ssak_debug_posconv_direct": (i32, [vp, vp, vp, vp, vp, i32, i32, i32, i32, i32, i32, i32, vp, sz, vp]),
         "ssak_debug_posconv_wgrad": (i32, [vp, vp, vp, i32, i32, i32, i32, i32, vp, sz, vp]),
         "ssak_debug_posconv_weight_bwd": (i32, [vp, vp, vp, vp, vp, vp, i32, i32, i32, vp]),
+        "ssak_debug_posconv_prepare_frag": (i32, [vp, vp, vp, vp, vp, i32, i32, i32, vp]),
+        "ssak_debug_posconv_frag": (i32, [vp, vp, i32, i32, i32, vp]),
+        "ssak_debug_colsum": (i32, [vp, i32, i32, vp, vp, sz, vp]),
+        "ssak_debug_head_workspace_bytes": (sz, [i32, i32]),
+        "ssak_debug_head_fwd": (i32, [vp, vp, vp, vp, vp, i32, i32, i32, C.c_uint64, C.c_uint32, f32, vp]),
+        "ssak_debug_head_bwd": (i32, [vp, vp, vp, vp, vp, i32, i32, i32, C.c_uint64, C.c_uint32, f32, vp, sz, vp]),
         "ssak_debug_conv0_bwd_workspace_bytes": (sz, [i32, i32, i32]),
         "ssak_debug_conv0_bwd": (i32, [vp, vp, vp, vp, vp, vp, vp, vp, vp, i32, i32, i32, i32, vp, sz, vp]),
         "ssak_debug_conv0_wgrad_workspace_bytes": (sz, [i32, i32, i32]),
@@ -952,6 +958,48 @@
     check(lib.ssak_debug_posconv_weight_bwd(ptr(dwf), ptr(g), ptr(v), ptr(norms), ptr(dg), ptr(dv), H, G, K, stream()))
 
 
+def debug_posconv_prepare_frag(g: torch.Tensor, v: torch.Tensor, G: int):
+    H, cg, K = v.shape
+    nan = float("nan")
+    wff = torch.full((H * K * cg,), nan, dtype=torch.bfloat16, device=v.device)
+    wbf = torch.full((H * K * cg,), nan, dtype=torch.bfloat16, device=v.device)
+    norms = torch.full(((2 + H) * K,), nan, dtype=torch.float32, device=v.device)
+    check(lib.ssak_debug_posconv_prepare_frag(ptr(g), ptr(v), ptr(wff), ptr(wbf), ptr(norms), H, G, K, stream()))
+    return wff, wbf, norms
+
+
+def debug_posconv_frag(w: torch.Tensor, H: int, G: int, K: int):
+    out = torch.full((w.numel(),), float("nan"), dtype=torch.bfloat16, device=w.device)
+    check(lib.ssak_debug_posconv_frag(ptr(w), ptr(out), H, G, K, stream()))
+    return out
+
+
+def debug_head_fwd(x: torch.Tensor, w: torch.Tensor, bias: torch.Tensor, *, seed: int = 0, site: int = 0, p: float = 0.0):
+    M, H = x.shape
+    V = w.shape[0]
+    logits = torch.full((M, V), float("nan"), dtype=torch.float32, device=x.device)
+    xf = torch.full((M, H), float("nan"), dtype=torch.bfloat16, device=x.device) if p > 0 else None
+    check(lib.ssak_debug_head_fwd(ptr(x), ptr(w), ptr(bias), ptr(xf), ptr(logits), M, H, V, seed, site, float(p), stream()))
+    return logits, xf
+
+
+def debug_head_bwd(dlogits: torch.Tensor, w: torch.Tensor, dbias: torch.Tensor, *, seed: int = 0, site: int = 0, p: float = 0.0):
+    M, V = dlogits.shape
+    H = w.shape[1]
+    dlog = torch.full((M, V), float("nan"), dtype=torch.bfloat16, device=w.device)
+    ga = torch.full((M, H), float("nan"), dtype=torch.bfloat16, device=w.device)
+    ws = torch.full((max(int(lib.ssak_debug_head_workspace_bytes(M, V)), 16),), 0xFF, dtype=torch.uint8, device=w.device)
+    check(lib.ssak_debug_head_bwd(ptr(dlogits), ptr(w), ptr(dlog), ptr(dbias), ptr(ga), M, H, V, seed, site, float(p), ptr(ws),
+                                  ws.numel(), stream()))
+    return dlog, ga
+
+
+def debug_colsum(x: torch.Tensor, out: torch.Tensor):
+    M, N = x.shape
+    ws = torch.full((min(64, (M + 31) // 32) * N * 4,), 0xFF, dtype=torch.uint8, device=x.device)
+    check(lib.ssak_debug_colsum(ptr(x), M, N, ptr(out), ptr(ws), ws.numel(), stream()))
+
+
 def debug_conv0_bwd_workspace(B: int, T: int, C_: int, device):
     nbytes = lib.ssak_debug_conv0_bwd_workspace_bytes(B, T, C_)
     return torch.full((max(int(nbytes), 16),), 0xFF, dtype=torch.uint8, device=device)
```
